# kluonj/HelFEM

Measured on AMD Instinct MI355X. Metric: scf_iteration_wall_time_fock_plus_geneig_nbf4230, lower is better.
Workload: dtype f64; 1 GPU; diatomic Z1=7 Z2=7 R=2.068 PBE, nelem=5 nnodes=15 nquad=75 lmmax=[20,20] (Nbf=4230, Nang=61, Nrad=70), XC grid 92x13, symmetry blocks [1380, 1470, 1380]: J+XC Fock build + eig_gsym_sub + density per step; parallelism=shard1, density=occupied orbitals of the core Hamiltonian

## Files before the change

helfem_amd/__init__.py:

```python
import ctypes
import os

import numpy as np

_HERE = os.path.dirname(os.path.abspath(__file__))
_LIB_PATH = os.environ.get("HELFEM_AMD_LIB") or os.path.join(_HERE, "lib", "libhelfem_amd.so")
_lib = None

c_double_p = ctypes.POINTER(ctypes.c_double)
c_int_p = ctypes.POINTER(ctypes.c_int)
c_i64_p = ctypes.POINTER(ctypes.c_int64)


class hfg_diatomic_desc(ctypes.Structure):
    _fields_ = [("Z1", ctypes.c_int), ("Z2", ctypes.c_int), ("Rhalf", ctypes.c_double), ("primbas", ctypes.c_int),
                ("nnodes", ctypes.c_int), ("nquad", ctypes.c_int), ("bval", c_double_p), ("nbval", ctypes.c_int),
                ("lval", c_int_p), ("mval", c_int_p), ("nang", ctypes.c_int), ("lpad", ctypes.c_int)]


class hfg_model_pot(ctypes.Structure):
    _fields_ = [("kind", ctypes.c_int), ("Z", ctypes.c_int), ("d", ctypes.c_double), ("H", ctypes.c_double)]


class hfg_atomic_desc(ctypes.Structure):
# ... 870 lines not shown

def xc_rs_kind(x_func):
    f = lib().hfg_xc_rs_kind
    f.argtypes = [ctypes.c_int]
    f.restype = ctypes.c_int
    return int(f(int(x_func)))


def scf_set_iguess(iguess):
    _check(lib().hfg_scf_set_iguess(int(iguess)))


def scf_diatomic(Z1, Z2, Rbond, lmmax, nelem, nnodes, method, nquad=0, Rmax=40.0, igrid=4, zexp=1.0, lpad=10, ldft=0,
                 mdft=0, symmetry=1, maxit=50, convthr=1e-7, verbose=0, ctx=None, M=1, occs=None, readocc=-1):
    ctx = ctx or default_context()
    L = lib()
    L.hfg_scf_diatomic.argtypes = [ctypes.c_void_p, ctypes.c_int, ctypes.c_int, ctypes.c_double, c_int_p, ctypes.c_int,
                                   ctypes.c_int, ctypes.c_int, ctypes.c_int, ctypes.c_double, ctypes.c_int,
                                   ctypes.c_double, ctypes.c_int, ctypes.c_char_p, ctypes.c_int, ctypes.c_int,
                                   ctypes.c_int, ctypes.c_int, ctypes.c_int, ctypes.c_double, ctypes.c_int, c_double_p]
    out = np.zeros(12)
    lm = (ctypes.c_int * len(lmmax))(*lmmax)
    scf_set_occupations(occs, readocc)
    try:
        _check(L.hfg_scf_diatomic(ctx.h, Z1, Z2, Rbond, lm, len(lmmax), nelem, nnodes, nquad, Rmax, igrid, zexp, lpad,
                                  method.encode(), ldft, mdft, symmetry, M, maxit, convthr, verbose, _p(out)))
    finally:
        scf_set_occupations(None)
    keys = ["Etot", "Ekin", "Epot", "Ecoul", "Exx", "Exc", "Enucr"]
    r = dict(zip(keys, out[:7]))
    r["iterations"] = int(out[7])
    r["converged"] = (out[7] - int(out[7])) > 0.25
    r["tJ"], r["tK"], r["tXC"], r["tdiag"] = out[8:12]
    return r


def scf_run_atomic(Z, lmax, mmax, nelem, nnodes, method="HF", ctx=None, check_only=False, E=None, C=None, extras=None, **kw):
    o = hfg_scf_options()
    _check(lib().hfg_scf_options_default(ctypes.byref(o), 1))
    o.Z1, o.lmax, o.mmax, o.nelem, o.nnodes = int(Z), int(lmax), int(mmax), int(nelem), int(nnodes)
    o.method = method.encode()
    o.verbose = 0
    o.save = b""
    for k, v in kw.items():
        if not hasattr(o, k):
            raise TypeError("hfg_scf_options has no field %s" % k)
        setattr(o, k, v.encode() if isinstance(v, str) else v)
    x = None
    if extras is not None:
        x = hfg_scf_atomic_extras()
        _check(lib().hfg_scf_atomic_extras_default(ctypes.byref(x)))
        for k, v in extras.items():
            if not hasattr(x, k):
                raise TypeError("hfg_scf_atomic_extras has no field %s" % k)
            setattr(x, k, v)
    xp = ctypes.byref(x) if x is not None else None
    if check_only:
        _check(lib().hfg_scf_options_check_ex(ctypes.byref(o), xp))
        return None
    ctx = ctx or default_context()
    r = hfg_scf_result()
    _check(lib().hfg_scf_run_ex(ctx.h, ctypes.byref(o), xp, ctypes.byref(r), _p(E) if E is not None else None,
                                _p(C) if C is not None else None))
    out = dict((f[0], getattr(r, f[0])) for f in hfg_scf_result._fields_)
    out["Econf"] = x.Econf if x is not None else 0.0
    return out


def scf_set_occupations(occs=None, readocc=-1):
    L = lib()
    L.hfg_scf_set_occupations.argtypes = [ctypes.c_int, ctypes.c_int, ctypes.c_int, ctypes.POINTER(ctypes.c_int)]
    if occs is None:
        _check(L.hfg_scf_set_occupations(0, 0, 0, None))
        return
    a = np.ascontiguousarray(np.asarray(occs, dtype=np.int32))
    _check(L.hfg_scf_set_occupations(int(readocc), a.shape[0], a.shape[1], a.ctypes.data_as(ctypes.POINTER(ctypes.c_int))))


def scf_atomic(Z, lmax, mmax, nelem, nnodes, method, Q=0, nquad=0, Rmax=40.0, igrid=4, zexp=2.0, ldft=0, mdft=0,
               symmetry=1, maxit=50, convthr=1e-7, verbose=0, ctx=None, M=1, maverage=False, occs=None, readocc=-1):
    ctx = ctx or default_context()
    L = lib()
    L.hfg_scf_atomic.argtypes = [ctypes.c_void_p] + [ctypes.c_int] * 7 + [ctypes.c_double, ctypes.c_int,
                                ctypes.c_double, ctypes.c_char_p] + [ctypes.c_int] * 6 + [ctypes.c_double,
                                ctypes.c_int, c_double_p]
    out = np.zeros(12)
    scf_set_occupations(occs, readocc)
    try:
        _check(L.hfg_scf_atomic(ctx.h, Z, Q, lmax, mmax, nelem, nnodes, nquad, Rmax, igrid, zexp, method.encode(), ldft,
                                mdft, symmetry, M, 1 if maverage else 0, maxit, convthr, verbose, _p(out)))
    finally:
        scf_set_occupations(None)
    keys = ["Etot", "Ekin", "Epot", "Ecoul", "Exx", "Exc", "Enucr"]
    r = dict(zip(keys, out[:7]))
    r["iterations"] = int(out[7])
    r["converged"] = (out[7] - int(out[7])) > 0.25
    r["tJ"], r["tK"], r["tXC"], r["tdiag"] = out[8:12]
    return r


class DeviceDIIS(object):

    def __init__(self, ctx, N, nspin, order=5, diiseps=1e-2, diisthr=1e-3, mode=0):
        self.h = None
        self.ctx, self.N, self.nspin, self.order, self.n = ctx, int(N), int(nspin), int(order), int(N)
        h = ctypes.c_void_p()
        _check(lib().hfg_diis_create(ctx.h, self.N, self.nspin, self.order, float(diiseps), float(diisthr), int(mode), ctypes.byref(h)))
        self.h = h

    def close(self):
        if self.h:
            if self.ctx.h:
                lib().hfg_diis_destroy(self.h)
            self.h = None

    def __del__(self):
        try:
            self.close()
        except Exception:
            pass

    @staticmethod
    def _dp(t):
        return ctypes.c_void_p(t.data_ptr()) if t is not None else None

    def _mat(self, t, cols, what):
        if t is None:
            return None
        if not (t.is_cuda and t.is_contiguous() and str(t.dtype) == "torch.float64" and t.numel() >= self.N * cols):
            raise ValueError("DeviceDIIS: %s must be a contiguous float64 tensor on the device with at least %d x %d elements"
                             % (what, self.N, cols))
        return t

    def set_metric(self, S, Sinvh):
        n = Sinvh.numel() // self.N
        if n * self.N != Sinvh.numel():
            raise ValueError("DeviceDIIS.set_metric: Sinvh is N x n")
        _check(lib().hfg_diis_set_metric_devptr(self.h, self._dp(self._mat(S, self.N, "S")), self._dp(self._mat(Sinvh, n, "Sinvh")), n))
        self.n = n

    def set_blocks(self, m_idx):
        ptr, idx = scf._blocks(m_idx or [])
        _check(lib().hfg_diis_set_blocks(self.h, len(m_idx or []), ptr.ctypes.data_as(c_i64_p), idx.ctypes.data_as(c_i64_p)))

    def update(self, E, Fa, Pa, Ca=None, nocca=0, Fb=None, Pb=None, Cb=None, noccb=0):
        if self.nspin == 2 and (Fb is None or Pb is None):
            raise ValueError("DeviceDIIS.update: nspin = 2 needs Fb and Pb")
        if self.nspin == 1 and (Fb is not None or Pb is not None):
            raise ValueError("DeviceDIIS.update: nspin = 1 takes one spin")
        err = ctypes.c_double()
        _check(lib().hfg_diis_update_devptr(self.h, float(E), self._dp(self._mat(Fa, self.N, "Fa")), self._dp(self._mat(Pa, self.N, "Pa")),
                                            self._dp(self._mat(Ca, int(nocca), "Ca")), int(nocca) if Ca is not None else 0,
                                            self._dp(self._mat(Fb, self.N, "Fb")), self._dp(self._mat(Pb, self.N, "Pb")),
                                            self._dp(self._mat(Cb, int(noccb), "Cb")), int(noccb) if Cb is not None else 0,
                                            ctypes.byref(err)))
        return err.value

    def solve(self, Fa, Fb=None):
        if self.nspin == 2 and Fb is None:
            raise ValueError("DeviceDIIS.solve: nspin = 2 needs Fb")
        dropped = ctypes.c_int()
        _check(lib().hfg_diis_solve_devptr(self.h, self._dp(self._mat(Fa, self.N, "Fa")), self._dp(self._mat(Fb, self.N, "Fb")),
                                           ctypes.byref(dropped)))
        return dropped.value

    @property
    def size(self):
        return int(lib().hfg_diis_size(self.h))

    def _get(self, which, count):
        out = np.zeros(max(count, 1))
        _check(lib().hfg_diis_get(self.h, which, _p(out), count))
        return out[:count]

    @property
    def B(self):
        k = self.size
        return self._get(0, k * k).reshape(k, k)

    @property
    def T(self):
        k = self.size
        return self._get(1, k * k).reshape(k, k)

    @property
    def weights(self):
        return self._get(2, self.size)

    @property
    def error(self):
        n = self.n
        return self._get(3, self.nspin * n * n).reshape(self.nspin, n, n).transpose(0, 2, 1)


def _refuse_out_of_scope(who, rohf, cuhf, readocc, maverage, dampfock):
    bad = [name for name, on in (("ROHF", rohf), ("CUHF", cuhf), ("readocc", readocc is not None and int(readocc) >= 0),
                                 ("maverage", maverage), ("dampfock", float(dampfock) != 1.0)) if on]
    if bad:
        raise NotImplementedError("%s.run: %s not supported by the step objects; use the SCF drivers (scf_diatomic, scf_atomic, "
                                  "scf_run_atomic)" % (who, ", ".join(bad)))


class DeviceSCFStep(object):

    def __init__(self, basis, x_func, c_func, ldft, mdft, nocc, symmetry=1, device=0, rank=0, nranks=1,
                 dens_thr=1e-12, kfrac=0.0, device_tei=False, fock_shard="auto"):
        self.nocc = int(nocc)
        self._setup(basis, x_func, c_func, ldft, mdft, symmetry, device, rank, nranks, dens_thr, kfrac, device_tei, fock_shard)
        f64 = dict(dtype=self.torch.float64, device=self.dev)
        L, N = lib(), self.N
        self.Fc = self.torch.zeros(int(L.hfg_fock_compact_size(basis.h)), **f64)
        self.scal = self.torch.zeros(3, **f64)
        self.F = self.torch.zeros(N * N, **f64)
        self.E = self.torch.zeros(N, **f64)
        self.C = self.torch.zeros(N * N, **f64)
        self.P = self.torch.zeros(N * N, **f64)
        nb = int(L.hfg_eig_block_buf_size(len(self.blocks), self.blk_ptr.ctypes.data_as(c_i64_p)))
        self.blockbuf = self.torch.zeros(nb, **f64)
        if self.kfrac != 0.0:
            self.K = self.torch.zeros(N * N, **f64)
            self.Pa = self.torch.zeros(N * N, **f64)

    def _setup(self, basis, x_func, c_func, ldft, mdft, symmetry, device, rank, nranks, dens_thr, kfrac, device_tei, fock_shard):
        import torch
        self.torch = torch
        self.basis = basis
        self.x_func, self.c_func, self.thr = int(x_func), int(c_func), float(dens_thr)
        self.dev = torch.device("cuda", device)
        torch.cuda.set_device(self.dev)
        self.ctx = Context(device, stream=torch.cuda.current_stream(self.dev).cuda_stream)
        self.ctx.set_shard(rank, nranks)
        self.rank, self.nranks = int(rank), int(nranks)
        self.fock_shard = os.environ.get("HELFEM_FOCK_SHARD", fock_shard)
        if device_tei:
            basis.compute_tei(float(kfrac) != 0.0, device=True, ctx=self.ctx)
        basis.upload(ldft, mdft, ctx=self.ctx)
        L = lib()
        L.hfg_fock_compact_size.restype = ctypes.c_int64
        L.hfg_eig_block_buf_size.restype = ctypes.c_int64
        L.hfg_fock_compact_dev.argtypes = [ctypes.c_void_p, ctypes.c_void_p, ctypes.c_int, ctypes.c_int, ctypes.c_void_p,
                                           ctypes.c_void_p, ctypes.c_void_p, ctypes.c_double]
        N = basis.Nbf()
        self.N = N
        self.blocks = basis.get_sym_idx(symmetry)
        self.blk_ptr, self.blk_idx = scf._blocks(self.blocks)
        blockid = np.zeros(N, dtype=np.int32)
        for ib, b in enumerate(self.blocks):
            blockid[b] = ib
        self.blockid = torch.from_numpy(blockid).to(self.dev)
        self.ctx.set_fock_blocks(basis, self.blockid.data_ptr())
        self.H0 = None
        self.Sinvh = None
        self.kfrac = float(kfrac)
        self.have_C = False
        self.have_density = False
        if self.kfrac != 0.0:
            L.hfg_exchange_occ_dev.argtypes = [ctypes.c_void_p, ctypes.c_void_p, ctypes.c_void_p, ctypes.c_void_p, ctypes.c_int64,
                                               ctypes.c_void_p]
            L.hfg_exchange_dev.argtypes = [ctypes.c_void_p, ctypes.c_void_p, ctypes.c_void_p, ctypes.c_void_p]

    def _ptr(self, t):
        return ctypes.c_void_p(t.data_ptr())

    def set_matrices(self, H0, Sinvh):
        t = self.torch
        self.H0 = t.from_numpy(np.asfortranarray(H0).ravel(order="F").copy()).to(self.dev)
        self.ctx.fix_sinvh(None)
        self.Sinvh = t.from_numpy(np.asfortranarray(Sinvh).ravel(order="F").copy()).to(self.dev)
        self.ctx.fix_sinvh(self.Sinvh.data_ptr())

    def set_density(self, P, C=None):
        self.P.copy_(self.torch.from_numpy(np.asfortranarray(P).ravel(order="F").copy()))
        self.have_density = True
        self.have_C = C is not None
        if C is not None:
            self.C[:self.N * self.nocc].copy_(self.torch.from_numpy(np.asfortranarray(C[:, :self.nocc]).ravel(order="F").copy()))

    def exchange(self):
        self.torch.mul(self.P, 0.5, out=self.Pa)
        if self.have_C:
            _check(lib().hfg_exchange_occ_dev(self.ctx.h, self.basis.h, self._ptr(self.Pa), self._ptr(self.C),
                                              ctypes.c_int64(self.nocc), self._ptr(self.K)))
        else:
            _check(lib().hfg_exchange_dev(self.ctx.h, self.basis.h, self._ptr(self.Pa), self._ptr(self.K)))

    def fock_partial(self):
        _check(lib().hfg_fock_compact_dev(self.ctx.h, self.basis.h, self.x_func, self.c_func, self._ptr(self.P),
                                          self._ptr(self.Fc), self._ptr(self.scal), self.thr))

    def fock_finish(self):
        _check(lib().hfg_fock_finish_dev(self.ctx.h, self.basis.h, self._ptr(self.Fc), self._ptr(self.H0),
                                         self._ptr(self.blockid), self._ptr(self.F)))

    def eig_partial(self):
        _check(lib().hfg_eig_blocks_dev(self.ctx.h, ctypes.c_int64(self.N), self._ptr(self.F), self._ptr(self.Sinvh),
                                        len(self.blocks), self.blk_ptr.ctypes.data_as(c_i64_p),
                                        self.blk_idx.ctypes.data_as(c_i64_p), self._ptr(self.blockbuf)))

    def eig_finish(self):
        _check(lib().hfg_eig_assemble_dev(self.ctx.h, ctypes.c_int64(self.N), len(self.blocks),
                                          self.blk_ptr.ctypes.data_as(c_i64_p), self.blk_idx.ctypes.data_as(c_i64_p),
                                          self._ptr(self.blockbuf), self._ptr(self.E), self._ptr(self.C)))

    def density(self):
        _check(lib().hfg_form_density_dev(self.ctx.h, ctypes.c_int64(self.N), ctypes.c_int64(self.N), self._ptr(self.C),
                                          ctypes.c_int64(self.nocc), self._ptr(self.P)))
        self.have_density = True

    def step(self, allreduce=None, exchange_blocks=None):
        shard_fock = self.nranks > 1 and self.fock_shard == "always"
        if self.nranks > 1 and not shard_fock:
            self.ctx.set_shard(0, 1)
        self.fock_partial()
        if self.nranks > 1 and not shard_fock:
            self.ctx.set_shard(self.rank, self.nranks)
        if allreduce is not None and (shard_fock or self.nranks == 1):
            allreduce(self.Fc)
            allreduce(self.scal)
        self.fock_finish()
        if self.kfrac != 0.0:
            self.exchange()
            if allreduce is not None:
                allreduce(self.K)
            self.F.add_(self.K, alpha=self.kfrac)
        self.eig_partial()
        if exchange_blocks is not None:
            exchange_blocks(self.blockbuf, len(self.blocks))
        elif allreduce is not None:
            allreduce(self.blockbuf)
        self.eig_finish()
        self.density()
        self.have_C = True

    def _whole_shard(self, fn):
        if self.nranks > 1:
            self.ctx.set_shard(0, 1)
        try:
            fn()
        finally:
            if self.nranks > 1:
                self.ctx.set_shard(self.rank, self.nranks)

    def _fock_stage(self, allreduce):
        shard_fock = self.nranks > 1 and self.fock_shard == "always"
        if shard_fock or self.nranks == 1:
            self.fock_partial()
            if allreduce is not None:
                allreduce(self.Fc)
                allreduce(self.scal)
        else:
            self._whole_shard(self.fock_partial)
        self.fock_finish()
        if self.kfrac != 0.0:
            self.exchange()
            if allreduce is not None:
                allreduce(self.K)
            self._add_exchange()

    def _add_exchange(self):
        self.F.add_(self.K, alpha=self.kfrac)

    def _eig_stage(self, allreduce, exchange_blocks):
        self.eig_partial()
        if exchange_blocks is not None:
            exchange_blocks(self.blockbuf, len(self.blocks))
        elif allreduce is not None:
            allreduce(self.blockbuf)
        self.eig_finish()

    def _coulomb_energy_matrix(self, P):
        if getattr(self, "J", None) is None:
            self.J = self.torch.zeros(self.N * self.N, dtype=self.torch.float64, device=self.dev)
        self._whole_shard(lambda: _check(lib().hfg_coulomb_dev(self.ctx.h, self.basis.h, self._ptr(P), self._ptr(self.J))))
        return self.J

    def _energy_terms(self):
        t = self.torch
        J = self._coulomb_energy_matrix(self.P)
        terms = [t.dot(self.P, self.H0), t.dot(self.P, J)]
        terms.append(t.dot(self.Pa, self.K) if self.kfrac != 0.0 else t.zeros((), dtype=t.float64, device=self.dev))
        return terms

    def energy(self, Enucr=0.0):
        t = self.torch
        v = t.stack(self._energy_terms() + [self.scal[0]]).cpu().numpy()
        r = dict(E1=float(v[0]), Ecoul=0.5 * float(v[1]), Exx=self._exx_factor() * float(v[2]), Exc=float(v[3]), Enucr=float(Enucr))
        r["Etot"] = r["E1"] + r["Ecoul"] + r["Exx"] + r["Exc"] + r["Enucr"]
        return r

    def _exx_factor(self):
        return self.kfrac

    def _nspin(self):
        return 1

    def _density_stage(self):
        self.density()
        self.P.mul_(2.0)
        self.have_C = True

    def _core_guess(self, allreduce, exchange_blocks):
        self.F.copy_(self.H0)
        self._eig_stage(allreduce, exchange_blocks)
        self._density_stage()

    def _diis_update(self, diis, E):
        if getattr(self, "Pa", None) is None:
            self.Pa = self.torch.zeros(self.N * self.N, dtype=self.torch.float64, device=self.dev)
        self.torch.mul(self.P, 0.5, out=self.Pa)
        if self.have_C:
            return diis.update(E, self.F, self.Pa, self.C, self.nocc)
        return diis.update(E, self.F, self.Pa)

    def _diis_solve(self, diis):
        diis.solve(self.F)

    def run(self, S, maxit=50, convthr=1e-7, Enucr=0.0, allreduce=None, exchange_blocks=None, diis=None, callback=None,
            rohf=False, cuhf=False, readocc=None, maverage=False, dampfock=1.0):
        _refuse_out_of_scope(type(self).__name__, rohf, cuhf, readocc, maverage, dampfock)
        if self.H0 is None:
            raise RuntimeError("run: set_matrices first")
        t = self.torch
        if diis is None:
            diis = DeviceDIIS(self.ctx, self.N, self._nspin())
            dS = t.from_numpy(np.asfortranarray(S, dtype=np.float64).ravel(order="F").copy()).to(self.dev)
            diis.set_metric(dS, self.Sinvh)
            if len(self.blocks) > 1:
                diis.set_blocks(self.blocks)
        if not self.have_density:
            self._core_guess(allreduce, exchange_blocks)
        trace, Eold, res, converged, it = [], 0.0, None, False, 0
        for it in range(1, int(maxit) + 1):
            self._fock_stage(allreduce)
            res = self.energy(Enucr)
            maxerr = self._diis_update(diis, res["Etot"])
            dE = res["Etot"] - Eold
            Eold = res["Etot"]
            trace.append((res["Etot"], maxerr))
            if callback is not None:
                callback(it, res["Etot"], maxerr)
            if maxerr < convthr and abs(dE) < convthr:
                converged = True
                break
            self._diis_solve(diis)
            self._eig_stage(allreduce, exchange_blocks)
            self._density_stage()
        res = dict(res or {})
        res.update(iterations=it, converged=converged, trace=trace)
        return res

    def numpy(self, t, shape):
        return t.cpu().numpy().reshape(shape, order="F")


class DeviceUSCFStep(DeviceSCFStep):

    def __init__(self, basis, x_func, c_func, ldft, mdft, nocc, symmetry=1, device=0, rank=0, nranks=1,
                 dens_thr=1e-12, kfrac=0.0, device_tei=False, fock_shard="auto"):
        self.nela, self.nelb = int(nocc[0]), int(nocc[1])
        if self.nela < 1 or self.nelb < 0:
            raise ValueError("DeviceUSCFStep: nocc = (nela >= 1, nelb >= 0)")
        self._setup(basis, x_func, c_func, ldft, mdft, symmetry, device, rank, nranks, dens_thr, kfrac, device_tei, fock_shard)
        t, N, L = self.torch, self.N, lib()
        f64 = dict(dtype=t.float64, device=self.dev)
        self.nc = int(L.hfg_fock_compact_size(basis.h))
        self.Fc = t.zeros(int(L.hfg_fock_compact_pol_size(basis.h)), **f64)
        self.scal = t.zeros(3, **f64)
        for name in ("Pa", "Pb", "Fa", "Fb", "Ca", "Cb"):
            setattr(self, name, t.zeros(N * N, **f64))
        self.Ea, self.Eb = t.zeros(N, **f64), t.zeros(N, **f64)
        if self.nranks > 1:
            nb = int(L.hfg_eig_block_buf_size(len(self.blocks), self.blk_ptr.ctypes.data_as(c_i64_p)))
            self.blockbuf_a, self.blockbuf_b = t.zeros(nb, **f64), t.zeros(nb, **f64)
        self.kbatch = False
        if self.kfrac != 0.0:
            self.K = t.zeros(2 * N * N, **f64)
            self.Ka, self.Kb = self.K[:N * N], self.K[N * N:]
            self.kbatch = {r["name"]: r["value"] for r in tuning_table()}["HELFEM_USCF_KBATCH"] == "on"
            if self.kbatch:
                self.Pab, self.Cab = t.zeros(2 * N * N, **f64), t.zeros(2 * N * N, **f64)
                self._nocc = np.array([self.nela, self.nelb], dtype=np.int64)

    def _spins(self):
        return ((self.Pa, self.Fa, self.Ea, self.Ca, self.nela), (self.Pb, self.Fb, self.Eb, self.Cb, self.nelb))

    def set_density(self, Pa, Pb, Ca=None, Cb=None):
        as_dev = lambda M: self.torch.from_numpy(np.asfortranarray(M).ravel(order="F").copy())
        self.Pa.copy_(as_dev(Pa))
        self.Pb.copy_(as_dev(Pb))
        self.have_density = True
        self.have_C = Ca is not None and (Cb is not None or self.nelb == 0)
        if self.have_C:
            self.Ca[:self.N * self.nela].copy_(as_dev(Ca[:, :self.nela]))
            if self.nelb:
                self.Cb[:self.N * self.nelb].copy_(as_dev(Cb[:, :self.nelb]))

    def exchange(self):
        if self.kbatch:
            N2 = self.N * self.N
            self.Pab[:N2].copy_(self.Pa)
            self.Pab[N2:].copy_(self.Pb)
            if self.have_C:
                self.Cab[:N2].copy_(self.Ca)
                self.Cab[N2:].copy_(self.Cb)
                _check(lib().hfg_exchange_occ_batch_devptr(self.ctx.h, self.basis.h, 2, self._ptr(self.Pab), self._ptr(self.Cab),
                                                           self._nocc.ctypes.data_as(c_i64_p), self.N, self._ptr(self.K)))
            else:
                _check(lib().hfg_exchange_batch_devptr(self.ctx.h, self.basis.h, 2, self._ptr(self.Pab), self._ptr(self.K)))
            return
        for (P, _, _, C, nocc), K in zip(self._spins(), (self.Ka, self.Kb)):
            if nocc == 0:
                K.zero_()
            elif self.have_C:
                _check(lib().hfg_exchange_occ_dev(self.ctx.h, self.basis.h, self._ptr(P), self._ptr(C), ctypes.c_int64(nocc),
                                                  self._ptr(K)))
            else:
                _check(lib().hfg_exchange_dev(self.ctx.h, self.basis.h, self._ptr(P), self._ptr(K)))

    def fock_partial(self):
        _check(lib().hfg_fock_compact_pol_devptr(self.ctx.h, self.basis.h, self.x_func, self.c_func, self._ptr(self.Pa),
                                                 self._ptr(self.Pb), self._ptr(self.Fc), self._ptr(self.scal), self.thr))

    def fock_finish(self):
        _check(lib().hfg_fock_finish_pol_devptr(self.ctx.h, self.basis.h, self._ptr(self.Fc), self._ptr(self.H0),
                                                self._ptr(self.blockid), self._ptr(self.Fa), self._ptr(self.Fb)))

    def eig_pair(self):
        _check(lib().hfg_eig_gsym_sub_pair_devptr(self.ctx.h, ctypes.c_int64(self.N), self._ptr(self.Fa), self._ptr(self.Fb),
                                                  self._ptr(self.Sinvh), len(self.blocks), self.blk_ptr.ctypes.data_as(c_i64_p),
                                                  self.blk_idx.ctypes.data_as(c_i64_p), self._ptr(self.Ea), self._ptr(self.Ca),
                                                  self._ptr(self.Eb), self._ptr(self.Cb)))

    def eig_partial(self):
        for (_, F, _, _, _), buf in zip(self._spins(), (self.blockbuf_a, self.blockbuf_b)):
            _check(lib().hfg_eig_blocks_dev(self.ctx.h, ctypes.c_int64(self.N), self._ptr(F), self._ptr(self.Sinvh),
                                            len(self.blocks), self.blk_ptr.ctypes.data_as(c_i64_p),
                                            self.blk_idx.ctypes.data_as(c_i64_p), self._ptr(buf)))

    def eig_finish(self):
        for (_, _, E, C, _), buf in zip(self._spins(), (self.blockbuf_a, self.blockbuf_b)):
            _check(lib().hfg_eig_assemble_dev(self.ctx.h, ctypes.c_int64(self.N), len(self.blocks),
                                              self.blk_ptr.ctypes.data_as(c_i64_p), self.blk_idx.ctypes.data_as(c_i64_p),
                                              self._ptr(buf), self._ptr(E), self._ptr(C)))

    def density(self):
        for P, _, _, C, nocc in self._spins():
            if nocc == 0:
                P.zero_()
                continue
            _check(lib().hfg_form_density_dev(self.ctx.h, ctypes.c_int64(self.N), ctypes.c_int64(self.N), self._ptr(C),
                                              ctypes.c_int64(nocc), self._ptr(P)))
        self.have_density = True

    def step(self, allreduce=None, exchange_blocks=None):
        shard_fock = self.nranks > 1 and self.fock_shard == "always"
        if self.nranks > 1 and not shard_fock:
            self.ctx.set_shard(0, 1)
        self.fock_partial()
        if self.nranks > 1 and not shard_fock:
            self.ctx.set_shard(self.rank, self.nranks)
        if allreduce is not None and (shard_fock or self.nranks == 1):
            allreduce(self.Fc)
            allreduce(self.scal)
        self.fock_finish()
        if self.kfrac != 0.0:
            self.exchange()
            if allreduce is not None:
                allreduce(self.K)
            self.Fa.add_(self.Ka, alpha=self.kfrac)
            self.Fb.add_(self.Kb, alpha=self.kfrac)
        if self.nranks == 1:
            self.eig_pair()
        else:
            self.eig_partial()
            for buf in (self.blockbuf_a, self.blockbuf_b):
                if exchange_blocks is not None:
                    exchange_blocks(buf, len(self.blocks))
                elif allreduce is not None:
                    allreduce(buf)
            self.eig_finish()
        self.density()
        self.have_C = True

    def _add_exchange(self):
        self.Fa.add_(self.Ka, alpha=self.kfrac)
        self.Fb.add_(self.Kb, alpha=self.kfrac)

    def _eig_stage(self, allreduce, exchange_blocks):
        if self.nranks == 1:
            self.eig_pair()
            return
        self.eig_partial()
        for buf in (self.blockbuf_a, self.blockbuf_b):
            if exchange_blocks is not None:
                exchange_blocks(buf, len(self.blocks))
            elif allreduce is not None:
                allreduce(buf)
        self.eig_finish()

    def _energy_terms(self):
        t = self.torch
        if getattr(self, "Pt", None) is None:
            self.Pt = t.zeros(self.N * self.N, dtype=t.float64, device=self.dev)
        t.add(self.Pa, self.Pb, out=self.Pt)
        J = self._coulomb_energy_matrix(self.Pt)
        terms = [t.dot(self.Pt, self.H0), t.dot(self.Pt, J)]
        terms.append(t.dot(self.Pa, self.Ka) + t.dot(self.Pb, self.Kb) if self.kfrac != 0.0
                     else t.zeros((), dtype=t.float64, device=self.dev))
        return terms

    def _exx_factor(self):
        return 0.5 * self.kfrac

    def _nspin(self):
        return 2

    def _density_stage(self):
        self.density()
        self.have_C = True

    def _core_guess(self, allreduce, exchange_blocks):
        self.Fa.copy_(self.H0)
        self.Fb.copy_(self.H0)
        self._eig_stage(allreduce, exchange_blocks)
        self._density_stage()

    def _diis_update(self, diis, E):
        if self.have_C:
            return diis.update(E, self.Fa, self.Pa, self.Ca, self.nela, self.Fb, self.Pb, self.Cb if self.nelb else None, self.nelb)
        return diis.update(E, self.Fa, self.Pa, Fb=self.Fb, Pb=self.Pb)

    def _diis_solve(self, diis):
        diis.solve(self.Fa, self.Fb)
```

helfem_amd/csrc/hip/common.h:

```cpp
#pragma once
#include <hip/hip_runtime.h>
#include <cstdint>
#include <cstring>
#include <map>
#include <stdexcept>
#include <string>
#include <vector>

#include "../../../include/helfem_gpu.h"
#include "../host/atomic_basis.h"
#include "../host/diatomic_basis.h"
#include "../host/tuning.h"
#include "workspace_owner.h"

namespace hfg {
using helfem::TrdMode, helfem::tuning;

void set_error(const std::string &msg);

#define HFG_HIP_CHECK(expr)                                                                          \
  do {                                                                                               \
    hipError_t _e = (expr);                                                                          \
    if (_e != hipSuccess)                                                                            \
      throw std::runtime_error(std::string("HIP error: ") + hipGetErrorString(_e) + " in " + #expr + \
                               " (" + __FILE__ + ":" + std::to_string(__LINE__) + ")");              \
  } while (0)

template <typename T>
struct DevBuf {
  T *p = nullptr;
  size_t n = 0;
  DevBuf() {}
  DevBuf(const DevBuf &) = delete;
  DevBuf &operator=(const DevBuf &) = delete;
  ~DevBuf() { release(); }
  void release() {
    if (p) (void)hipFree(p);
    p = nullptr;
    n = 0;
  }
  void resize(size_t count) {
    if (count <= n) return;
    release();
    HFG_HIP_CHECK(hipMalloc((void **)&p, count * sizeof(T)));
    n = count;
  }
  void upload(const std::vector<T> &h, hipStream_t s) {
    resize(h.size() ? h.size() : 1);
    if (h.size()) HFG_HIP_CHECK(hipMemcpyAsync(p, h.data(), h.size() * sizeof(T), hipMemcpyHostToDevice, s));
  }
};

template <typename T>
bool upload_cached(DevBuf<T> &buf, std::vector<T> &cache, const std::vector<T> &h, hipStream_t s) {
  if (buf.p && cache.size() == h.size() && buf.n >= h.size() &&
      (h.empty() || memcmp((const void *)cache.data(), (const void *)h.data(), h.size() * sizeof(T)) == 0))
    return false;
  HFG_HIP_CHECK(hipStreamSynchronize(s));
  cache = h;
  buf.upload(cache, s);
  return true;
}

struct ProfEntry {
  double ms = 0.0;
  int64_t launches = 0;
  std::vector<std::pair<hipEvent_t, hipEvent_t> > pending;
};

}

struct hfg_dev_tables;

struct hfg_ctx {
  int device = 0;
  hipStream_t stream = nullptr;
  bool own_stream = false;
  hipStream_t side_stream = nullptr;
  hipEvent_t side_ev[2] = {nullptr, nullptr};
  hipStream_t side();
  bool avoid_side = false;
  void drop_side();
  int shard_rank = 0, shard_n = 1;
  const double *fixed_sinvh = nullptr;
  unsigned long fixed_gen = 0;
  void fix_sinvh(const double *p) {
    fixed_sinvh = p;
    fixed_gen++;
  }
  hfg::DevBuf<int> fock_need, fock_gneed;
  const hfg_dev_tables *fock_need_tables = nullptr;
  int fock_need_A = 0, fock_need_G = 0;
  bool profiling = false;
  std::map<std::string, hfg::ProfEntry> prof;
  std::vector<hipEvent_t> event_pool;
  hfg::DevBuf<double> ws[8];
  double *pinned = nullptr;
  size_t pinned_bytes = 0;
  hfg::WorkspaceOwner<hfg::WS_CTX_SLOTS> work;

  void *pinned_buf(size_t bytes);
  hipEvent_t get_event();
  void prof_begin(const char *name);
  void prof_end(const char *name);
  void prof_collect();
};

struct hfg_basis {
  int kind = 0;
  helfem::diatomic::TwoDBasis b;
  helfem::atomic::TwoDBasis ab;
  hfg_dev_tables *dev = nullptr;
  hfg_dev_tables *dev_rs = nullptr;
  int dev_device = -1;
  hfg::DevBuf<double> dev_tei;
  bool tei_on_device = false;
  hfg::DevBuf<double> dev_rs_tei, dev_rs_disj;
  bool rs_on_device = false;

  size_t Nbf() const { return kind ? ab.Nbf() : b.Nbf(); }
  size_t Ndummy() const { return kind ? ab.Nbf() : b.Ndummy(); }
  size_t Nrad() const { return kind ? ab.Nrad() : b.Nrad(); }
  size_t Nang() const { return kind ? ab.Nang() : b.Nang(); }
  size_t Nel() const { return kind ? ab.Nel() : b.Nel(); }
  size_t max_Nprim() const { return kind ? ab.max_Nprim() : b.max_Nprim(); }
  bool have_tei() const { return tei_on_device || (kind ? ab.have_tei : b.have_tei); }
};

namespace hfg {
struct GemmTask {
  const double *A;
  const double *B;
  double *C;
  int M, N, K, lda, ldb, ldc;
  int tA = 0, tB = 0;
  double alpha = 1.0, beta = 0.0;
  int sym = 0;
  int over = 0;
  const int *amap = nullptr, *cmap = nullptr;
};
static_assert(sizeof(GemmTask) == 96, "GemmTask is compared bytewise: keep it free of padding");

struct ProfScope {
  hfg_ctx *c;
  const char *n;
  ProfScope(hfg_ctx *ctx, const char *name) : c(ctx), n(name) {
    if (c->profiling) c->prof_begin(n);
  }
  ~ProfScope() {
    if (c->profiling) c->prof_end(n);
  }
};
}
```

helfem_amd/csrc/hip/eig.hip:

```cpp
#include "internal.h"
#include "wave.h"
#include "../host/eigsel_count.h"
#include <cstdlib>
#include <cstring>

namespace hfg {

constexpr int MAXB = 8;
struct EigBatch {
  int nblk;
  int n[MAXB];
  double *A[MAXB];
  double *d[MAXB];
  double *e[MAXB];
  double *tau[MAXB];
  double *v[MAXB];
  double *pp[MAXB];
  double *dots[MAXB];
  double *Z[MAXB];
  int nz[MAXB];
  double *rot[MAXB];
  int *sweeps[MAXB];
  long rotcap[MAXB];
};

constexpr int TRD_NCS = 8;

__global__ void k_gather_block(const double *__restrict__ F, const double *__restrict__ S, int N,
                               const int64_t *__restrict__ rows, const int64_t *__restrict__ cols, int n,
                               double *__restrict__ Fb, double *__restrict__ Xb) {
  int i = blockIdx.x * blockDim.x + threadIdx.x;
  int j = blockIdx.y;
  if (i >= n) return;
  Fb[(size_t)j * n + i] = F[(size_t)rows[j] * N + rows[i]];
  Xb[(size_t)j * n + i] = S[(size_t)cols[j] * N + rows[i]];
}

__global__ void k_col_support(const double *__restrict__ S, int N, const int64_t *__restrict__ rows, int n,
                              int *__restrict__ flag) {
  int c = blockIdx.x;
  int any = 0;
  for (int i = threadIdx.x; i < n; i += blockDim.x)
    if (S[(size_t)c * N + rows[i]] != 0.0) any = 1;
  any = __syncthreads_or(any);
  if (threadIdx.x == 0) flag[c] = any;
}

__device__ inline void householder_of_column(const double *__restrict__ A, int n, int k, double *vsh, double *red,
                                             double &tau, double &beta) {
  const int m = n - k - 1;
  const double *x = A + (size_t)k * n + k + 1;
  double s = 0.0;
  for (int i = 1 + threadIdx.x; i < m; i += blockDim.x) s += x[i] * x[i];
  s = wave_sum(s);
  int nwave = blockDim.x / 64;
  if ((threadIdx.x & 63) == 0) red[threadIdx.x >> 6] = s;
  __syncthreads();
  double xn2 = 0.0;
  for (int w = 0; w < nwave; w++) xn2 += red[w];
  double alpha = x[0];
  double scale;
  if (xn2 == 0.0) {
    tau = 0.0;
    beta = alpha;
    scale = 0.0;
  } else {
    double nrm = sqrt(alpha * alpha + xn2);
    beta = (alpha >= 0.0) ? -nrm : nrm;
    tau = (beta - alpha) / beta;
    scale = 1.0 / (alpha - beta);
  }
  for (int i = threadIdx.x; i < m; i += blockDim.x) vsh[i] = (i == 0) ? 1.0 : x[i] * scale;
  __syncthreads();
}

__global__ __launch_bounds__(256) void k_trd_gemv(EigBatch b, int k) {
  extern __shared__ double sh[];
  const int blk = blockIdx.y;
  const int n = b.n[blk];
  if (k > n - 3) return;
  const int m = n - k - 1;
  const int nrs = (m + 63) / 64;
  const int rs = blockIdx.x / TRD_NCS, cs = blockIdx.x % TRD_NCS;
  if (rs >= nrs) return;
  double *A = b.A[blk];
  double *vsh = sh;
  double *red = sh + n;
  double tau, beta;
  householder_of_column(A, n, k, vsh, red, tau, beta);
  if (blockIdx.x == 0) {
    for (int i = threadIdx.x; i < m; i += blockDim.x) b.v[blk][i] = vsh[i];
    if (threadIdx.x == 0) {
      b.tau[blk][k] = tau;
      b.e[blk][k] = beta;
      b.d[blk][k] = A[(size_t)k * n + k];
    }
  }
  const int cchunk = (m + TRD_NCS - 1) / TRD_NCS;
  const int c0 = cs * cchunk, c1 = min(m, c0 + cchunk);
  const int wave = threadIdx.x >> 6, lane = threadIdx.x & 63;
  const int row = rs * 64 + lane;
  double acc = 0.0;
  if (row < m) {
    const double *a = A + (size_t)(k + 1) * n + (k + 1) + row;
    for (int c = c0 + wave; c < c1; c += 4) acc += a[(size_t)c * n] * vsh[c];
  }
  __syncthreads();
  red[wave * 64 + lane] = acc;
  __syncthreads();
  if (wave == 0) {
    double p = red[lane] + red[64 + lane] + red[128 + lane] + red[192 + lane];
    if (row < m) b.pp[blk][(size_t)cs * n + row] = p;
    double dv = (row < m) ? p * vsh[row] : 0.0;
    dv = wave_sum(dv);
    if (lane == 0) b.dots[blk][blockIdx.x] = dv;
  }
}

__global__ __launch_bounds__(256) void k_trd_update(EigBatch b, int k) {
  __shared__ double vr[64], vc[64], wr[64], wc[64];
  __shared__ double Ksh;
  const int blk = blockIdx.y;
  const int n = b.n[blk];
  if (k > n - 3) return;
  const int m = n - k - 1;
  const int nt = (m + 63) / 64;
  if ((int)blockIdx.x >= nt * nt) return;
  const int tr = blockIdx.x % nt, tc = blockIdx.x / nt;
  double *A = b.A[blk];
  const double tau = b.tau[blk][k];
  if (threadIdx.x == 0) {
    const int nrs = (m + 63) / 64;
    double s = 0.0;
    for (int i = 0; i < nrs * TRD_NCS; i++) s += b.dots[blk][i];
    Ksh = 0.5 * tau * tau * s;
  }
  __syncthreads();
  if (threadIdx.x < 128) {
    int which = threadIdx.x >> 6, l = threadIdx.x & 63;
    int idx = (which ? tc : tr) * 64 + l;
    double v = 0.0, w = 0.0;
    if (idx < m) {
      v = b.v[blk][idx];
      double p = 0.0;
      for (int cs = 0; cs < TRD_NCS; cs++) p += b.pp[blk][(size_t)cs * n + idx];
      w = tau * p - Ksh * v;
    }
    if (which) {
      vc[l] = v;
      wc[l] = w;
    } else {
      vr[l] = v;
      wr[l] = w;
    }
  }
  __syncthreads();
  const int lane = threadIdx.x & 63, wave = threadIdx.x >> 6;
  const int row = tr * 64 + lane;
  if (row < m) {
    double *a = A + (size_t)(k + 1) * n + (k + 1) + row;
    for (int c = wave; c < 64; c += 4) {
      int col = tc * 64 + c;
      if (col < m) a[(size_t)col * n] -= vr[lane] * wc[c] + wr[lane] * vc[c];
    }
  }
  if (blockIdx.x == 0) {
    for (int i = 1 + threadIdx.x; i < m; i += blockDim.x) A[(size_t)k * n + k + 1 + i] = b.v[blk][i];
  }
}

__global__ void k_trd_finish(EigBatch b) {
  int blk = blockIdx.x;
  if (threadIdx.x != 0) return;
  int n = b.n[blk];
  double *A = b.A[blk];
  if (n >= 2) {
    b.d[blk][n - 2] = A[(size_t)(n - 2) * n + (n - 2)];
    b.e[blk][n - 2] = A[(size_t)(n - 2) * n + (n - 1)];
    b.tau[blk][n - 2] = 0.0;
  }
  b.d[blk][n - 1] = A[(size_t)(n - 1) * n + (n - 1)];
  b.e[blk][n - 1] = 0.0;
}

__global__ void k_tql_values(EigBatch b) {
  int blk = blockIdx.x;
  if (threadIdx.x != 0) return;
  const int n = b.n[blk];
  double *d = b.d[blk], *e = b.e[blk];
  double *rot = b.rot[blk];
  int *sw = b.sweeps[blk];
  long nrot = 0;
  int nsw = 0;
  int status = 0;
  const long cap = b.rotcap[blk];
  for (int l = 0; l < n && !status; l++) {
    int iter = 0;
    int m;
    do {
      for (m = l; m + 1 < n; m++) {
        double dd = fabs(d[m]) + fabs(d[m + 1]);
        if (fabs(e[m]) <= 2.220446049250313e-16 * dd) break;
      }
      if (m != l) {
        if (iter++ == 300) {
          status = 1;
          break;
        }
        if (nrot + (m - l) > cap || 4 * (nsw + 1) + 2 >= 4 * 64 * n) {
          status = 2;
          break;
        }
        double g = (d[l + 1] - d[l]) / (2.0 * e[l]);
        double r = hypot(g, 1.0);
        g = d[m] - d[l] + e[l] / (g + (g >= 0.0 ? fabs(r) : -fabs(r)));
        double s = 1.0, c = 1.0, p = 0.0;
        int cnt = 0;
        bool under = false;
        int i;
        for (i = m - 1; i >= l; i--) {
          double f = s * e[i], bb = c * e[i];
          r = hypot(f, g);
          e[i + 1] = r;
          if (r == 0.0) {
            d[i + 1] -= p;
            e[m] = 0.0;
            under = true;
            break;
          }
          s = f / r;
          c = g / r;
          g = d[i + 1] - p;
          r = (d[i] - g) * s + 2.0 * c * bb;
          p = s * r;
          d[i + 1] = g + p;
          g = c * r - bb;
          rot[2 * (nrot + cnt)] = c;
          rot[2 * (nrot + cnt) + 1] = s;
          cnt++;
        }
        sw[2 + 4 * nsw + 0] = l;
        sw[2 + 4 * nsw + 1] = m;
        sw[2 + 4 * nsw + 2] = (int)(nrot & 0x7fffffff);
        sw[2 + 4 * nsw + 3] = cnt;
        nsw++;
        nrot += cnt;
        if (under) continue;
        d[l] -= p;
        e[l] = g;
        e[m] = 0.0;
      }
    } while (m != l);
  }
  sw[0] = nsw;
  sw[1] = status;
}

__global__ void k_set_identity(EigBatch b) {
  int blk = blockIdx.z;
  int n = b.n[blk];
  int i = blockIdx.x * blockDim.x + threadIdx.x, j = blockIdx.y;
  if (i < n && j < n) b.Z[blk][(size_t)j * n + i] = (i == j) ? 1.0 : 0.0;
}

__global__ void k_tql_apply(EigBatch b) {
  int blk = blockIdx.y;
  int n = b.n[blk];
  int k = blockIdx.x * blockDim.x + threadIdx.x;
  if (k >= n) return;
  double *Z = b.Z[blk] + k;
  const double *rot = b.rot[blk];
  const int *sw = b.sweeps[blk];
  int nsw = sw[0];
  long off = 0;
  for (int q = 0; q < nsw; q++) {
    int m = sw[2 + 4 * q + 1], cnt = sw[2 + 4 * q + 3];
    double hi = Z[(size_t)m * n];
    int i = m - 1;
    for (int t = 0; t < cnt; t++, i--) {
      double c = rot[2 * (off + t)], s = rot[2 * (off + t) + 1];
      double lo = Z[(size_t)i * n];
      Z[(size_t)(i + 1) * n] = s * lo + c * hi;
      hi = c * lo - s * hi;
    }
    Z[(size_t)(i + 1) * n] = hi;
    off += cnt;
  }
}

template <int NR>
__global__ __launch_bounds__(256) void k_backtransform(EigBatch b) {
  int blk = blockIdx.y;
  int n = b.n[blk];
  int col = blockIdx.x * 4 + (threadIdx.x >> 6);
  int lane = threadIdx.x & 63;
  if (col >= b.nz[blk]) return;
  const double *A = b.A[blk];
  const double *tau = b.tau[blk];
  double *z = b.Z[blk] + (size_t)col * n;
  double zr[NR];
#pragma unroll
  for (int r = 0; r < NR; r++) {
    int i = lane + 64 * r;
    zr[r] = (i < n) ? z[i] : 0.0;
  }
  for (int k = n - 3; k >= 0; k--) {
    double t = tau[k];
    if (t == 0.0) continue;
    const double *v = A + (size_t)k * n;
    double s = 0.0;
    double vr[NR];
#pragma unroll
    for (int r = 0; r < NR; r++) {
      int i = lane + 64 * r;
      double vi = 0.0;
      if (i == k + 1) vi = 1.0;
      else if (i > k + 1 && i < n) vi = v[i];
      vr[r] = vi;
      s += vi * zr[r];
    }
    s = wave_sum(s);
    s *= t;
#pragma unroll
    for (int r = 0; r < NR; r++) zr[r] -= s * vr[r];
  }
#pragma unroll
  for (int r = 0; r < NR; r++) {
    int i = lane + 64 * r;
    if (i < n) z[i] = zr[r];
  }
}

__global__ __launch_bounds__(256) void k_backtransform_lds(EigBatch b) {
  extern __shared__ double sh[];
  int blk = blockIdx.y;
  int n = b.n[blk];
  int wave = threadIdx.x >> 6, lane = threadIdx.x & 63;
  int col = blockIdx.x * 4 + wave;
  if (col >= b.nz[blk]) return;
  const double *A = b.A[blk];
  const double *tau = b.tau[blk];
  double *z = b.Z[blk] + (size_t)col * n;
  double *zs = sh + (size_t)wave * n;
  for (int i = lane; i < n; i += 64) zs[i] = z[i];
  for (int k = n - 3; k >= 0; k--) {
    double t = tau[k];
    if (t == 0.0) continue;
    const double *v = A + (size_t)k * n;
    double s = 0.0;
    for (int i = k + 1 + lane; i < n; i += 64) s += ((i == k + 1) ? 1.0 : v[i]) * zs[i];
    s = wave_sum(s);
    s *= t;
    for (int i = k + 1 + lane; i < n; i += 64) zs[i] -= s * ((i == k + 1) ? 1.0 : v[i]);
  }
  for (int i = lane; i < n; i += 64) z[i] = zs[i];
}

constexpr int RANK_SEG = 8;
__global__ __launch_bounds__(256) void k_rank(const double *__restrict__ E, int n, int *__restrict__ rank) {
  __shared__ double sE[256];
  const int i = blockIdx.x * 256 + threadIdx.x;
  const double ei = (i < n) ? E[i] : 0.0;
  const int seg = (n + RANK_SEG - 1) / RANK_SEG;
  const int j0 = blockIdx.y * seg, j1 = min(n, j0 + seg);
  int r = 0;
  for (int c = j0; c < j1; c += 256) {
    __syncthreads();
    sE[threadIdx.x] = (c + (int)threadIdx.x < j1) ? E[c + threadIdx.x] : 0.0;
    __syncthreads();
    const int m = min(256, j1 - c);
    if (m == 256) {
#pragma unroll 16
      for (int jj = 0; jj < 256; jj++) {
        const double ej = sE[jj];
        r += (ej < ei) || (ej == ei && c + jj < i);
      }
    } else {
      for (int jj = 0; jj < m; jj++) {
        const double ej = sE[jj];
        r += (ej < ei) || (ej == ei && c + jj < i);
      }
    }
  }
  if (i < n && r) atomicAdd(&rank[i], r);
}
static void launch_rank(hfg_ctx *ctx, const double *E, int n, int *rank) {
  HFG_HIP_CHECK(hipMemsetAsync(rank, 0, sizeof(int) * n, ctx->stream));
  hipLaunchKernelGGL(k_rank, dim3((n + 255) / 256, RANK_SEG), dim3(256), 0, ctx->stream, E, n, rank);
}

__global__ void k_scatter_cols(const double *__restrict__ Cb, int nrow, int ncol, const int64_t *__restrict__ rows,
                               const int *__restrict__ rank, int coff, const double *__restrict__ Eb, int ldc,
                               double *__restrict__ Cout, double *__restrict__ Eout) {
  int i = blockIdx.x * blockDim.x + threadIdx.x;
  int j = blockIdx.y;
  if (i >= nrow) return;
  int c = rank[coff + j];
  size_t r = rows ? (size_t)rows[i] : (size_t)i;
  Cout[(size_t)c * ldc + r] = Cb[(size_t)j * nrow + i];
  if (i == 0) Eout[c] = Eb[j];
}

__global__ void k_take_lowest(const double *__restrict__ Z, const double *__restrict__ E, int n, int nev, const int *__restrict__ rank,
                              double *__restrict__ Zs, double *__restrict__ Ws) {
  int i = blockIdx.x * blockDim.x + threadIdx.x;
  int j = blockIdx.y;
  int c = rank[j];
  if (i >= n || c >= nev) return;
  Zs[(size_t)c * n + i] = Z[(size_t)j * n + i];
  if (i == 0) Ws[c] = E[j];
}

constexpr int BT_KB = 64;

__global__ void k_bt_extract(EigBatch b, double *const *__restrict__ Vx) {
  const int blk = blockIdx.z;
  const int n = b.n[blk];
  const int j = blockIdx.y;
  const int g = blockIdx.x * blockDim.x + threadIdx.x;
  if (j >= n || g >= n) return;
  double v = 0.0;
  if (j <= n - 3) {
    if (g == j + 1) v = 1.0;
    else if (g > j + 1) v = b.A[blk][(size_t)j * n + g];
  }
  Vx[blk][(size_t)j * n + g] = v;
}

constexpr int BT_PW = 2 * BT_KB;
constexpr int BT_WREP = 4;
__global__ __launch_bounds__(256) void k_bt_wpair(EigBatch b, double *const *__restrict__ Wpart, double *const *__restrict__ W,
                                                  double *const *__restrict__ Cc, int S, int GS, int npair, int pair,
                                                  int mirror) {
  __shared__ double sC[BT_KB][BT_KB + 1];
  __shared__ double s1[4][BT_KB];
  const int blk = blockIdx.y;
  const int n = b.n[blk];
  const int j0 = pair * BT_PW;
  if (j0 > n - 3) return;
  const int kb1 = min(BT_KB, n - 2 - (j0 + BT_KB));
  const int tid = threadIdx.x, cl = tid >> 6, i = tid & 63;
  if (kb1 > 0) {
    constexpr int NE = BT_KB * BT_KB / 256;
    double c[NE];
#pragma unroll
    for (int u = 0; u < NE; u++) c[u] = 0.0;
    for (int sl = 0; sl < GS; sl++) {
      const double *src = Cc[blk] + ((size_t)sl * npair + pair) * BT_KB * BT_KB + tid;
#pragma unroll
      for (int u = 0; u < NE; u++) c[u] += src[256 * u];
    }
#pragma unroll
    for (int u = 0; u < NE; u++) {
      const int t = tid + 256 * u;
      sC[t % BT_KB][t / BT_KB] = c[u];
    }
  }
  const size_t tot = (size_t)BT_PW * n;
  double a0[BT_WREP], a1[BT_WREP];
#pragma unroll
  for (int rep = 0; rep < BT_WREP; rep++) {
    const int col = (blockIdx.x * BT_WREP + rep) * 4 + cl;
    a0[rep] = 0.0;
    a1[rep] = 0.0;
    if (col < n) {
      for (int sl = 0; sl < S; sl++) {
        a0[rep] += Wpart[blk][(size_t)sl * tot + (size_t)col * BT_PW + i];
        a1[rep] += Wpart[blk][(size_t)sl * tot + (size_t)col * BT_PW + BT_KB + i];
      }
    }
  }
  if (mirror) {
    const int kb0 = min(BT_KB, n - 2 - j0);
#pragma unroll
    for (int rep = 0; rep < BT_WREP; rep++) {
      const int col = (blockIdx.x * BT_WREP + rep) * 4 + cl;
      __syncthreads();
      s1[cl][i] = (i < kb0) ? a0[rep] : 0.0;
      __syncthreads();
      if (col < n) {
        double r1 = 0.0;
        if (kb1 > 0 && i < kb1) {
          double corr = 0.0;
          for (int j = 0; j < kb0; j++) corr += sC[j][i] * s1[cl][j];
          r1 = a1[rep] - corr;
        }
        W[blk][(size_t)col * BT_PW + i] = a0[rep];
        W[blk][(size_t)col * BT_PW + BT_KB + i] = r1;
      }
    }
    return;
  }
#pragma unroll
  for (int rep = 0; rep < BT_WREP; rep++) {
    const int col = (blockIdx.x * BT_WREP + rep) * 4 + cl;
    __syncthreads();
    s1[cl][i] = (kb1 > 0 && i < kb1) ? a1[rep] : 0.0;
    __syncthreads();
    if (col < n) {
      double r0 = a0[rep];
      if (kb1 > 0) {
        double corr = 0.0;
        for (int j = 0; j < kb1; j++) corr += sC[i][j] * s1[cl][j];
        r0 -= corr;
      }
      W[blk][(size_t)col * BT_PW + i] = r0;
      W[blk][(size_t)col * BT_PW + BT_KB + i] = (kb1 > 0 && i < kb1) ? a1[rep] : 0.0;
    }
  }
}

constexpr int BT_GS = 4;
__global__ __launch_bounds__(64) void k_bt_T(EigBatch b, double *const *__restrict__ G, double *const *__restrict__ T,
                                             int P) {
  __shared__ double sT[BT_KB][BT_KB + 1];
  __shared__ double sG[BT_KB][BT_KB + 1];
  __shared__ double sg[BT_KB];
  const int blk = blockIdx.y, p = blockIdx.x;
  const int n = b.n[blk];
  const int j0 = p * BT_KB;
  if (j0 > n - 3) return;
  const int kb = min(BT_KB, n - 2 - j0);
  double *Tp = T[blk] + (size_t)p * BT_KB * BT_KB;
  const int t = threadIdx.x;
  for (int c0 = 0; c0 < BT_KB; c0 += 16) {
    double g[16];
#pragma unroll
    for (int u = 0; u < 16; u++) g[u] = 0.0;
#pragma unroll
    for (int sl = 0; sl < BT_GS; sl++) {
      const double *src = G[blk] + ((size_t)sl * P + p) * BT_KB * BT_KB + (size_t)c0 * BT_KB + t;
#pragma unroll
      for (int u = 0; u < 16; u++) g[u] += src[(size_t)u * BT_KB];
    }
#pragma unroll
    for (int u = 0; u < 16; u++) {
      sG[c0 + u][t] = g[u];
      sT[t][c0 + u] = 0.0;
    }
  }
  __shared__ double stau[BT_KB];
  stau[t] = (t < kb) ? b.tau[blk][j0 + t] : 0.0;
  __syncthreads();
  for (int i = 0; i < kb; i++) {
    const double ti = stau[i];
    sg[t] = (t < i) ? sG[i][t] : 0.0;
    __syncthreads();
    if (t < i) {
      double acc0 = 0.0, acc1 = 0.0, acc2 = 0.0, acc3 = 0.0;
#pragma unroll
      for (int k = 0; k < BT_KB; k += 4) {
        acc0 += sT[t][k] * sg[k];
        acc1 += sT[t][k + 1] * sg[k + 1];
        acc2 += sT[t][k + 2] * sg[k + 2];
        acc3 += sT[t][k + 3] * sg[k + 3];
      }
      sT[t][i] = -ti * ((acc0 + acc1) + (acc2 + acc3));
    }
    if (t == i) sT[i][i] = ti;
    __syncthreads();
  }
  for (int c = 0; c < BT_KB; c++) Tp[(size_t)c * BT_KB + t] = sT[t][c];
}

struct EigWork : Workspace {
  GemmHow full_how;
  std::vector<int64_t> asm_rows;
  DevBuf<long long> asm_rows_dev;
  bool folded = false;
  DevBuf<double> Y[MAXB];
  DevBuf<GemmTask> btslabR, btupdR;
  std::vector<GemmTask> h_btslabR, h_btupdR;
  DevBuf<double> A[MAXB], d[MAXB], e[MAXB], tau[MAXB], v[MAXB], pp[MAXB], dots[MAXB], Z[MAXB], rot[MAXB];
  DevBuf<double> Zs[MAXB], Ws[MAXB];
  DevBuf<int> selrank;
  DevBuf<int> sweeps[MAXB];
  DevBuf<int> ibuf1, ibuf2;
  DevBuf<GemmTask> gtasks, bttasks, btslab, btgram, btcpl, btupd;
  std::vector<GemmTask> h_gtasks, h_bttasks, h_btslab, h_btgram, h_btcpl, h_btupd;
  std::vector<double *> h_btptr;
  DevBuf<double> Vx[MAXB], G[MAXB], T[MAXB], VT[MAXB], Wb[MAXB], Wp[MAXB], Cc[MAXB];
  DevBuf<double *> btptr;
  bool used_dc = true;
  DevBuf<double> idx;
  const double *sup_S = nullptr;
  unsigned long sup_gen = 0;
  int sup_N = 0;
  std::vector<int64_t> sup_ptr, sup_idx;
};
static EigWork &work_for(hfg_ctx *ctx) { return ctx->work.get<EigWork>(WS_EIG); }

struct CopySlices {
  const double *src[16];
  double *dst[16];
  int n[16];
};
__global__ void k_copy_slices(CopySlices c) {
  const int q = blockIdx.y;
  for (int i = blockIdx.x * blockDim.x + threadIdx.x; i < c.n[q]; i += gridDim.x * blockDim.x) c.dst[q][i] = c.src[q][i];
}
static void copy_slices(hipStream_t s, const std::vector<const double *> &src, const std::vector<double *> &dst, const std::vector<int> &n) {
  for (size_t q0 = 0; q0 < src.size(); q0 += 16) {
    CopySlices c{};
    const int m = (int)std::min<size_t>(16, src.size() - q0);
    int nmax = 0;
    for (int q = 0; q < m; q++) {
      c.src[q] = src[q0 + q];
      c.dst[q] = dst[q0 + q];
      c.n[q] = n[q0 + q];
      nmax = std::max(nmax, n[q0 + q]);
    }
    if (nmax > 0) hipLaunchKernelGGL(k_copy_slices, dim3((nmax + 255) / 256, m), dim3(256), 0, s, c);
  }
}

struct TrPtrs {
  const double *src[MAXB];
  double *dst[MAXB];
  int n[MAXB];
};
__global__ __launch_bounds__(256) void k_transpose_batch(TrPtrs t) {
  __shared__ double tile[64][65];
  const int blk = blockIdx.z, n = t.n[blk];
  const int bi = blockIdx.x * 64, bj = blockIdx.y * 64;
  if (bi >= n || bj >= n) return;
  const int tx = threadIdx.x & 63, ty = threadIdx.x >> 6;
  for (int c = ty; c < 64; c += 4) {
    const int gm = bi + tx, gn = bj + c;
    tile[c][tx] = (gm < n && gn < n) ? t.src[blk][(size_t)gn * n + gm] : 0.0;
  }
  __syncthreads();
  for (int c = ty; c < 64; c += 4) {
    const int gm = bj + tx, gn = bi + c;
    if (gm < n && gn < n) t.dst[blk][(size_t)gn * n + gm] = tile[tx][c];
  }
}

static void bt_wy_setup(hfg_ctx *ctx, EigWork &w, const EigBatch &b, int nblk, const int *ns, int nmax, bool fold = false) {
  hipStream_t s = ctx->stream;
  const int P = (nmax - 3) / BT_KB + 1;
  const int NP = (P + 1) / 2;
  constexpr int BT_S = 6;
  std::vector<double *> ptrs(6 * (size_t)nblk);
  for (int k = 0; k < nblk; k++) {
    const int n = ns[k];
    w.Vx[k].resize((size_t)n * n);
    w.G[k].resize((size_t)BT_GS * P * BT_KB * BT_KB);
    w.T[k].resize((size_t)P * BT_KB * BT_KB);
    w.VT[k].resize((size_t)n * P * BT_KB);
    w.Wb[k].resize((size_t)BT_PW * n);
    w.Wp[k].resize((size_t)BT_S * BT_PW * n);
    w.Cc[k].resize((size_t)BT_GS * NP * BT_KB * BT_KB);
    ptrs[k] = w.Vx[k].p;
    ptrs[nblk + k] = w.G[k].p;
    ptrs[2 * nblk + k] = w.T[k].p;
    ptrs[3 * nblk + k] = w.Wp[k].p;
    ptrs[4 * nblk + k] = w.Wb[k].p;
    ptrs[5 * nblk + k] = w.Cc[k].p;
  }
  upload_cached(w.btptr, w.h_btptr, ptrs, s);
  GemmTask none;
  none.A = none.B = nullptr;
  none.C = nullptr;
  none.M = none.N = none.K = 0;
  none.lda = none.ldb = none.ldc = 1;
  auto kb_of = [&](int k, int p) { return std::max(0, std::min(BT_KB, ns[k] - 2 - p * BT_KB)); };
  auto chunk_of = [](int len, int parts) { return ((len + parts - 1) / parts + 15) / 16 * 16; };

  std::vector<GemmTask> gram((size_t)BT_GS * P * nblk, none), vt((size_t)P * nblk, none);
  for (int p = 0; p < P; p++)
    for (int k = 0; k < nblk; k++) {
      const int n = ns[k], j0 = p * BT_KB, kb = kb_of(k, p);
      if (kb <= 0) continue;
      const int r0 = j0 + 1, mr = n - r0;
      const double *Vp = w.Vx[k].p + (size_t)j0 * n + r0;
      const int chunk = chunk_of(mr, BT_GS);
      for (int sl = 0; sl < BT_GS; sl++) {
        GemmTask g = none;
        const int k0 = sl * chunk, kk = std::max(0, std::min(chunk, mr - k0));
        g.A = g.B = Vp + (kk > 0 ? k0 : 0);
        g.C = w.G[k].p + ((size_t)sl * P + p) * BT_KB * BT_KB;
        g.tA = 1;
        g.M = g.N = kb;
        g.K = kk;
        g.lda = g.ldb = n;
        g.ldc = BT_KB;
        gram[((size_t)sl * P + p) * nblk + k] = g;
      }
      const int rp = (p & ~1) * BT_KB + 1;
      GemmTask g = none;
      g.A = w.Vx[k].p + (size_t)j0 * n + rp;
      g.B = w.T[k].p + (size_t)p * BT_KB * BT_KB;
      g.C = w.VT[k].p + (size_t)j0 * n + rp;
      g.M = n - rp;
      g.N = g.K = kb;
      g.lda = n;
      g.ldb = BT_KB;
      g.ldc = n;
      vt[(size_t)p * nblk + k] = g;
    }
  upload_cached(w.btgram, w.h_btgram, gram, s);
  upload_cached(w.bttasks, w.h_bttasks, vt, s);

  std::vector<GemmTask> cpl((size_t)BT_GS * NP * nblk, none), slab((size_t)NP * BT_S * nblk, none), upd((size_t)NP * nblk, none);
  for (int g2 = 0; g2 < NP; g2++)
    for (int k = 0; k < nblk; k++) {
      const int n = ns[k], p0 = 2 * g2, j0 = p0 * BT_KB;
      const int kb0 = kb_of(k, p0), kb1 = (p0 + 1 < P) ? kb_of(k, p0 + 1) : 0;
      if (kb0 <= 0) continue;
      const int r0 = j0 + 1, mr = n - r0, kbp = kb0 + kb1;
      if (kb1 > 0) {
        const int r1 = j0 + BT_KB + 1, m1 = n - r1;
        const int chunk = chunk_of(m1, BT_GS);
        for (int sl = 0; sl < BT_GS; sl++) {
          GemmTask c = none;
          const int k0 = sl * chunk, kk = std::max(0, std::min(chunk, m1 - k0));
          c.A = w.Vx[k].p + (size_t)j0 * n + r1 + (kk > 0 ? k0 : 0);
          c.B = w.VT[k].p + (size_t)(j0 + BT_KB) * n + r1 + (kk > 0 ? k0 : 0);
          c.C = w.Cc[k].p + ((size_t)sl * NP + g2) * BT_KB * BT_KB;
          c.tA = 1;
          c.M = kb0;
          c.N = kb1;
          c.K = kk;
          c.lda = c.ldb = n;
          c.ldc = BT_KB;
          cpl[((size_t)sl * NP + g2) * nblk + k] = c;
        }
      }
      const int chunk = chunk_of(mr, BT_S);
      for (int sl = 0; sl < BT_S; sl++) {
        GemmTask q = none;
        const int k0 = sl * chunk, kk = std::max(0, std::min(chunk, mr - k0));
        q.A = w.Vx[k].p + (size_t)j0 * n + r0 + (kk > 0 ? k0 : 0);
        q.B = b.Z[k] + r0 + (kk > 0 ? k0 : 0);
        q.C = w.Wp[k].p + (size_t)sl * BT_PW * n;
        q.tA = 1;
        q.M = kbp;
        q.N = b.nz[k];
        q.K = kk;
        q.lda = q.ldb = n;
        q.ldc = BT_PW;
        slab[((size_t)g2 * BT_S + sl) * nblk + k] = q;
      }
      GemmTask u = none;
      u.A = w.VT[k].p + (size_t)j0 * n + r0;
      u.B = w.Wb[k].p;
      u.C = b.Z[k] + r0;
      u.M = mr;
      u.N = b.nz[k];
      u.K = kbp;
      u.lda = n;
      u.ldb = BT_PW;
      u.ldc = n;
      u.alpha = -1.0;
      u.beta = 1.0;
      upd[(size_t)g2 * nblk + k] = u;
    }
  upload_cached(w.btcpl, w.h_btcpl, cpl, s);
  upload_cached(w.btslab, w.h_btslab, slab, s);
  upload_cached(w.btupd, w.h_btupd, upd, s);
  if (fold) {
    std::vector<GemmTask> slabR((size_t)NP * BT_S * nblk, none), updR((size_t)NP * nblk, none);
    for (int g2 = 0; g2 < NP; g2++)
      for (int k = 0; k < nblk; k++) {
        const int n = ns[k], p0 = 2 * g2, j0 = p0 * BT_KB;
        const int kb0 = kb_of(k, p0), kb1 = (p0 + 1 < P) ? kb_of(k, p0 + 1) : 0;
        if (kb0 <= 0) continue;
        const int r0 = j0 + 1, mr = n - r0, kbp = kb0 + kb1;
        const int chunk = chunk_of(mr, BT_S);
        for (int sl = 0; sl < BT_S; sl++) {
          GemmTask q = none;
          const int k0 = sl * chunk, kk = std::max(0, std::min(chunk, mr - k0));
          q.A = w.VT[k].p + (size_t)j0 * n + r0 + (kk > 0 ? k0 : 0);
          q.B = w.Y[k].p + r0 + (kk > 0 ? k0 : 0);
          q.C = w.Wp[k].p + (size_t)sl * BT_PW * n;
          q.tA = 1;
          q.M = kbp;
          q.N = n;
          q.K = kk;
          q.lda = q.ldb = n;
          q.ldc = BT_PW;
          slabR[((size_t)g2 * BT_S + sl) * nblk + k] = q;
        }
        GemmTask u = none;
        u.A = w.Vx[k].p + (size_t)j0 * n + r0;
        u.B = w.Wb[k].p;
        u.C = w.Y[k].p + r0;
        u.M = mr;
        u.N = n;
        u.K = kbp;
        u.lda = n;
        u.ldb = BT_PW;
        u.ldc = n;
        u.alpha = -1.0;
        u.beta = 1.0;
        updR[(size_t)g2 * nblk + k] = u;
      }
    upload_cached(w.btslabR, w.h_btslabR, slabR, s);
    upload_cached(w.btupdR, w.h_btupdR, updR, s);
  }
}

static void bt_wy_prepare(hfg_ctx *ctx, EigWork &w, const EigBatch &b, int nblk, int nmax, bool on_side = false) {
  const int P = (nmax - 3) / BT_KB + 1;
  const bool use_side = (tuning().bt_side && !ctx->avoid_side) || on_side;
  hipStream_t main = ctx->stream, q = main;
  const bool prof = ctx->profiling;
  if (use_side) {
    q = ctx->side();
    HFG_HIP_CHECK(hipEventRecord(ctx->side_ev[0], main));
    HFG_HIP_CHECK(hipStreamWaitEvent(q, ctx->side_ev[0], 0));
    ctx->profiling = false;
    ctx->stream = q;
  }
  try {
    double *const *dptr = w.btptr.p;
    hipLaunchKernelGGL(k_bt_extract, dim3((nmax + 255) / 256, nmax, nblk), dim3(256), 0, q, b, dptr);
    gemm_tasklist_dev(ctx, w.btgram.p, BT_GS * P * nblk, BT_KB, BT_KB, {GemmTile::T64});
    hipLaunchKernelGGL(k_bt_T, dim3(P, nblk), dim3(BT_KB), 0, q, b, dptr + nblk, dptr + 2 * nblk, P);
    gemm_tasklist_dev(ctx, w.bttasks.p, P * nblk, nmax, BT_KB, {GemmTile::T64});
    gemm_tasklist_dev(ctx, w.btcpl.p, BT_GS * ((P + 1) / 2) * nblk, BT_KB, BT_KB, {GemmTile::T64});
  } catch (...) {
    ctx->stream = main;
    ctx->profiling = prof;
    throw;
  }
  ctx->stream = main;
  ctx->profiling = prof;
  if (use_side) HFG_HIP_CHECK(hipEventRecord(ctx->side_ev[1], q));
}

static void bt_wy_apply(hfg_ctx *ctx, EigWork &w, const EigBatch &b, int nblk, int nmax) {
  hipStream_t s = ctx->stream;
  const int P = (nmax - 3) / BT_KB + 1, NP = (P + 1) / 2;
  constexpr int BT_S = 6;
  double *const *dptr = w.btptr.p;
  if (tuning().bt_side && !ctx->avoid_side) HFG_HIP_CHECK(hipStreamWaitEvent(s, ctx->side_ev[1], 0));
  for (int g = NP - 1; g >= 0; g--) {
    gemm_tasklist_dev(ctx, w.btslab.p + (size_t)g * BT_S * nblk, BT_S * nblk, BT_PW, nmax, {GemmTile::T64});
    hipLaunchKernelGGL(k_bt_wpair, dim3((nmax + 4 * BT_WREP - 1) / (4 * BT_WREP), nblk), dim3(256), 0, s, b, dptr + 3 * nblk, dptr + 4 * nblk,
                       dptr + 5 * nblk, BT_S, BT_GS, NP, g, 0);
    gemm_tasklist_dev(ctx, w.btupd.p + (size_t)g * nblk, nblk, nmax, nmax, {tuning().acc_tile != 128 ? GemmTile::T64 : GemmTile::T128,  true});
  }
  HFG_HIP_CHECK(hipGetLastError());
}

static void bt_wy_fold_x(hfg_ctx *ctx, EigWork &w, const EigBatch &b, int nblk, const int *ns, int nmax, const double *const *X) {
  const int P = (nmax - 3) / BT_KB + 1, NP = (P + 1) / 2;
  constexpr int BT_S = 6;
  hipStream_t main = ctx->stream, q = ctx->side();
  const bool prof = ctx->profiling;
  ctx->profiling = false;
  ctx->stream = q;
  try {
    TrPtrs t;
    for (int k = 0; k < MAXB; k++) {
      t.src[k] = k < nblk ? X[k] : nullptr;
      t.dst[k] = k < nblk ? w.Y[k].p : nullptr;
      t.n[k] = k < nblk ? ns[k] : 0;
    }
    hipLaunchKernelGGL(k_transpose_batch, dim3((nmax + 63) / 64, (nmax + 63) / 64, nblk), dim3(256), 0, q, t);
    double *const *dptr = w.btptr.p;
    for (int g = 0; g < NP; g++) {
      gemm_tasklist_dev(ctx, w.btslabR.p + (size_t)g * BT_S * nblk, BT_S * nblk, BT_PW, nmax, {GemmTile::T64});
      hipLaunchKernelGGL(k_bt_wpair, dim3((nmax + 4 * BT_WREP - 1) / (4 * BT_WREP), nblk), dim3(256), 0, q, b, dptr + 3 * nblk, dptr + 4 * nblk,
                         dptr + 5 * nblk, BT_S, BT_GS, NP, g, 1);
      gemm_tasklist_dev(ctx, w.btupdR.p + (size_t)g * nblk, nblk, nmax, nmax, {GemmTile::T64,  true});
    }
  } catch (...) {
    ctx->stream = main;
    ctx->profiling = prof;
    throw;
  }
  ctx->stream = main;
  ctx->profiling = prof;
  HFG_HIP_CHECK(hipGetLastError());
  HFG_HIP_CHECK(hipEventRecord(ctx->side_ev[1], q));
}

constexpr double EIGSEL_CROSS = 0.0;
static bool eigsel_takes_stein(int nblk, const int *ns, const int *nev) {
  const helfem::EigSel how = tuning().eigsel;
  if (how != helfem::EigSel::crossover) return how == helfem::EigSel::stein;
  long want = 0, all = 0;
  for (int i = 0; i < nblk; i++) {
    want += nev[i];
    all += ns[i];
  }
  return (double)want <= EIGSEL_CROSS * (double)all;
}
static void eig_sym_batch(hfg_ctx *ctx, EigWork &w, int nblk, const int *ns, const double *const *foldX = nullptr,
                          const int *nev = nullptr) {
  EigBatch b;
  b.nblk = nblk;
  int nmax = 0, nzmax = 0;
  const bool stein = nev && eigsel_takes_stein(nblk, ns, nev);
  for (int i = 0; i < nblk; i++) {
    int n = ns[i];
    nmax = std::max(nmax, n);
    b.n[i] = n;
    b.nz[i] = nev ? nev[i] : n;
    nzmax = std::max(nzmax, b.nz[i]);
    if (nev) {
      if (nev[i] < 1 || nev[i] > n) throw std::logic_error("eig_sym_batch: 1 <= nev <= n violated\n");
      w.Zs[i].resize((size_t)n * nev[i]);
      w.Ws[i].resize(nev[i]);
    }
    w.d[i].resize(n);
    w.e[i].resize(n);
    w.tau[i].resize(n);
    w.v[i].resize(n);
    w.pp[i].resize((size_t)TRD_NCS * n);
    w.dots[i].resize((size_t)TRD_NCS * ((n + 63) / 64) + 8);
    if (!stein) w.Z[i].resize((size_t)n * n);
    long cap = 3L * n * n + 1024;
    w.rot[i].resize(2 * (size_t)cap);
    w.sweeps[i].resize((size_t)4 * 64 * n + 8);
    b.rotcap[i] = cap;
    b.A[i] = w.A[i].p;
    b.d[i] = w.d[i].p;
    b.e[i] = w.e[i].p;
    b.tau[i] = w.tau[i].p;
    b.v[i] = w.v[i].p;
    b.pp[i] = w.pp[i].p;
    b.dots[i] = w.dots[i].p;
    b.Z[i] = stein ? nullptr : w.Z[i].p;
    b.rot[i] = w.rot[i].p;
    b.sweeps[i] = w.sweeps[i].p;
  }
  hipStream_t s = ctx->stream;
  const bool bt_wy = !tuning().bt_column && nmax >= 4 * BT_KB;
  if (tridiagonalize_takes_chain(nblk, ns)) {
    ctx->avoid_side = true;
    ctx->drop_side();
  }
  const bool fold = bt_wy && foldX != nullptr && tuning().bt_fold && !ctx->avoid_side;
  w.folded = fold;
  if (fold)
    for (int i = 0; i < nblk; i++) w.Y[i].resize((size_t)ns[i] * ns[i]);
  EigBatch bz = b;
  if (nev)
    for (int i = 0; i < nblk; i++) bz.Z[i] = w.Zs[i].p;
  if (bt_wy) bt_wy_setup(ctx, w, bz, nblk, ns, nmax, fold);
  {
    ProfScope ps(ctx, "eig_tridiag");
    if (tuning().trd_mode == TrdMode::unblocked) {
      size_t shb = (size_t)(nmax + 4 * 64 + 8) * sizeof(double);
      if (shb > 64 * 1024)
        HFG_HIP_CHECK(hipFuncSetAttribute((const void *)k_trd_gemv, hipFuncAttributeMaxDynamicSharedMemorySize, (int)shb));
      for (int k = 0; k <= nmax - 3; k++) {
        int m = nmax - k - 1;
        int nrs = (m + 63) / 64;
        hipLaunchKernelGGL(k_trd_gemv, dim3(nrs * TRD_NCS, nblk), dim3(256), shb, s, b, k);
        hipLaunchKernelGGL(k_trd_update, dim3(nrs * nrs, nblk), dim3(256), 0, s, b, k);
      }
      hipLaunchKernelGGL(k_trd_finish, dim3(nblk), dim3(64), 0, s, b);
    } else {
      double *Ap[MAXB], *dp[MAXB], *ep[MAXB], *tp[MAXB];
      for (int i = 0; i < nblk; i++) {
        Ap[i] = w.A[i].p;
        dp[i] = w.d[i].p;
        ep[i] = w.e[i].p;
        tp[i] = w.tau[i].p;
      }
      tridiagonalize_batch(ctx, nblk, ns, Ap, dp, ep, tp);
    }
  }
  if (bt_wy) bt_wy_prepare(ctx, w, b, nblk, nmax, fold);
  if (fold) bt_wy_fold_x(ctx, w, b, nblk, ns, nmax, foldX);
  if (stein) {
    ProfScope ps(ctx, "eig_tridiag_sel");
    w.used_dc = true;
    double *dp[MAXB], *ep[MAXB], *wp[MAXB], *zp[MAXB];
    for (int i = 0; i < nblk; i++) {
      dp[i] = w.d[i].p;
      ep[i] = w.e[i].p;
      wp[i] = w.Ws[i].p;
      zp[i] = w.Zs[i].p;
    }
    tridiag_sel_batch(ctx, nblk, ns, nev, dp, ep, wp, zp);
  } else {
    ProfScope ps(ctx, "eig_tridiag_solve");
    w.used_dc = !tuning().tridiag_ql;
    if (!w.used_dc) {
      hipLaunchKernelGGL(k_set_identity, dim3((nmax + 255) / 256, nmax, nblk), dim3(256), 0, s, b);
      hipLaunchKernelGGL(k_tql_values, dim3(nblk), dim3(64), 0, s, b);
      hipLaunchKernelGGL(k_tql_apply, dim3((nmax + 63) / 64, nblk), dim3(64), 0, s, b);
    } else {
      double *dp[MAXB], *ep[MAXB], *zp[MAXB];
      for (int i = 0; i < nblk; i++) {
        dp[i] = w.d[i].p;
        ep[i] = w.e[i].p;
        zp[i] = w.Z[i].p;
      }
      tridiag_dc_batch(ctx, nblk, ns, dp, ep, zp);
    }
    if (nev) {
      size_t off = 0;
      for (int i = 0; i < nblk; i++) off += ns[i] + 8;
      w.selrank.resize(off);
      off = 0;
      for (int i = 0; i < nblk; i++) {
        launch_rank(ctx, w.d[i].p, ns[i], w.selrank.p + off);
        hipLaunchKernelGGL(k_take_lowest, dim3((ns[i] + 255) / 256, ns[i]), dim3(256), 0, s, w.Z[i].p, w.d[i].p, ns[i], nev[i],
                           w.selrank.p + off, w.Zs[i].p, w.Ws[i].p);
        off += ns[i] + 8;
      }
    }
  }
  {
    ProfScope ps(ctx, "eig_backtransform");
    if (fold) {
      HFG_HIP_CHECK(hipStreamWaitEvent(s, ctx->side_ev[1], 0));
    } else if (bt_wy) {
      bt_wy_apply(ctx, w, bz, nblk, nmax);
    } else {
    dim3 grid((nzmax + 3) / 4, nblk);
    if (nmax <= 64 * 8)
      hipLaunchKernelGGL(k_backtransform<8>, grid, dim3(256), 0, s, bz);
    else if (nmax <= 64 * 24)
      hipLaunchKernelGGL(k_backtransform<24>, grid, dim3(256), 0, s, bz);
    else {
      size_t shb = (size_t)4 * nmax * sizeof(double);
      if (shb > 64 * 1024)
        HFG_HIP_CHECK(
            hipFuncSetAttribute((const void *)k_backtransform_lds, hipFuncAttributeMaxDynamicSharedMemorySize, (int)shb));
      hipLaunchKernelGGL(k_backtransform_lds, grid, dim3(256), shb, s, bz);
    }
    }
  }
  HFG_HIP_CHECK(hipGetLastError());
}

static void check_status(hfg_ctx *ctx, EigWork &w, int nblk) {
  if (w.used_dc) {
    if (dc_status(ctx) != 0) throw std::logic_error("Eigendecomposition failed!\n");
    trdp_check_status(ctx);
    return;
  }
  for (int i = 0; i < nblk; i++) {
    int st[2];
    HFG_HIP_CHECK(hipMemcpyAsync(st, w.sweeps[i].p, 2 * sizeof(int), hipMemcpyDeviceToHost, ctx->stream));
    HFG_HIP_CHECK(hipStreamSynchronize(ctx->stream));
    if (st[1] != 0) throw std::logic_error("Eigendecomposition failed!\n");
  }
}

void eig_sym_dev(hfg_ctx *ctx, int n, const double *dA, double *dE, double *dC) {
  EigWork &w = work_for(ctx);
  w.A[0].resize((size_t)n * n + 2);
  HFG_HIP_CHECK(hipMemcpyAsync(w.A[0].p, dA, sizeof(double) * n * n, hipMemcpyDeviceToDevice, ctx->stream));
  eig_sym_batch(ctx, w, 1, &n);
  DevBuf<int> &rank = w.ibuf1;
  rank.resize(n + 8);
  launch_rank(ctx, w.d[0].p, n, rank.p);
  hipLaunchKernelGGL(k_scatter_cols, dim3((n + 255) / 256, n), dim3(256), 0, ctx->stream, w.Z[0].p, n, n,
                     (const int64_t *)nullptr, rank.p, 0, w.d[0].p, n, dC, dE);
  check_status(ctx, w, 1);
}

void eig_sym_sel_dev(hfg_ctx *ctx, int n, const double *dA, int nev, double *dE, double *dC) {
  if (nev < 1) throw std::logic_error("eig_sym_sel: nev must be at least 1\n");
  if (n < 1) throw std::logic_error("eig_sym_sel: empty matrix\n");
  nev = std::min(nev, n);
  EigWork &w = work_for(ctx);
  w.A[0].resize((size_t)n * n + 2);
  HFG_HIP_CHECK(hipMemcpyAsync(w.A[0].p, dA, sizeof(double) * n * n, hipMemcpyDeviceToDevice, ctx->stream));
  eig_sym_batch(ctx, w, 1, &n, nullptr, &nev);
  HFG_HIP_CHECK(hipMemcpyAsync(dC, w.Zs[0].p, sizeof(double) * (size_t)n * nev, hipMemcpyDeviceToDevice, ctx->stream));
  HFG_HIP_CHECK(hipMemcpyAsync(dE, w.Ws[0].p, sizeof(double) * nev, hipMemcpyDeviceToDevice, ctx->stream));
  check_status(ctx, w, 1);
}

void eig_gsym_dev(hfg_ctx *ctx, int N, int n, const double *dF, const double *dS, double *dE, double *dC) {
  EigWork &w = work_for(ctx);
  w.A[0].resize((size_t)n * n + 2);
  DevBuf<double> &T1 = ctx->ws[0];
  DevBuf<double> &Ctmp = ctx->ws[1];
  T1.resize((size_t)N * n);
  Ctmp.resize((size_t)N * n);
  {
    ProfScope ps(ctx, "eig_reduce");
    gemm_dev(ctx, false, false, N, n, N, 1.0, dF, N, dS, N, 0.0, T1.p, N);
    gemm_dev(ctx, true, false, n, n, N, 1.0, dS, N, T1.p, N, 0.0, w.A[0].p, n);
  }
  eig_sym_batch(ctx, w, 1, &n);
  {
    ProfScope ps(ctx, "eig_backtransform");
    gemm_dev(ctx, false, false, N, n, n, 1.0, dS, N, w.Z[0].p, n, 0.0, Ctmp.p, N);
  }
  DevBuf<int> &rank = w.ibuf1;
  rank.resize(n + 8);
  launch_rank(ctx, w.d[0].p, n, rank.p);
  hipLaunchKernelGGL(k_scatter_cols, dim3((N + 255) / 256, n), dim3(256), 0, ctx->stream, Ctmp.p, N, n,
                     (const int64_t *)nullptr, rank.p, 0, w.d[0].p, N, dC, dE);
  check_status(ctx, w, 1);
}

size_t eig_block_buf_size(int nblk, const int64_t *blk_ptr) {
  size_t nmax = 0;
  for (int ib = 0; ib < nblk; ib++) nmax = std::max<size_t>(nmax, blk_ptr[ib + 1] - blk_ptr[ib]);
  return (size_t)nblk * (nmax * nmax + nmax);
}

static void eig_blocks_multi_dev(hfg_ctx *ctx, int N, int nF, const double *const *dFs, const double *dS, int nblk, const int64_t *blk_ptr,
                                 const int64_t *blk_idx, double *const *dBlockBufs, int nev = 0);
static int eig_num_cus(hfg_ctx *ctx) {
  static const int ncu = [&] {
    hipDeviceProp_t prop;
    return (hipGetDeviceProperties(&prop, ctx->device) == hipSuccess && prop.multiProcessorCount > 0) ? prop.multiProcessorCount : 256;
  }();
  return ncu;
}
void eig_blocks_dev(hfg_ctx *ctx, int N, const double *dF, const double *dS, int nblk, const int64_t *blk_ptr,
                    const int64_t *blk_idx, double *dBlockBuf) {
  eig_blocks_multi_dev(ctx, N, 1, &dF, dS, nblk, blk_ptr, blk_idx, &dBlockBuf);
}
static void eig_blocks_multi_dev(hfg_ctx *ctx, int N, int nF, const double *const *dFs, const double *dS, int nblk, const int64_t *blk_ptr,
                                 const int64_t *blk_idx, double *const *dBlockBufs, int nev) {
  EigWork &w = work_for(ctx);
  hipStream_t s = ctx->stream;
  if (blk_ptr[nblk] != N) throw std::logic_error("Symmetry mismatch in eig_gsym_sub\n");
  DevBuf<double> &idxbuf = w.idx;
  idxbuf.resize(2 * (size_t)N + 16);
  int64_t *drows = (int64_t *)idxbuf.p;
  int64_t *dcols = drows + N;
  for (int ib = 0; ib < nblk; ib++)
    if (blk_ptr[ib + 1] == blk_ptr[ib]) throw std::logic_error("eig_gsym_sub: empty symmetry block\n");
  const bool cached = ctx->fixed_sinvh && ctx->fixed_sinvh == dS && w.sup_S == dS && w.sup_gen == ctx->fixed_gen &&
                      w.sup_N == N &&
                      w.sup_ptr.size() == (size_t)nblk + 1 && std::equal(w.sup_ptr.begin(), w.sup_ptr.end(), blk_ptr) &&
                      w.sup_idx.size() == (size_t)N && std::equal(w.sup_idx.begin(), w.sup_idx.end(), blk_idx);
  if (!cached) {
    w.sup_S = nullptr;
    HFG_HIP_CHECK(hipMemcpyAsync(drows, blk_idx, sizeof(int64_t) * N, hipMemcpyHostToDevice, s));
    DevBuf<int> &flag = w.ibuf2;
    flag.resize((size_t)N * nblk + 8);
    for (int ib = 0; ib < nblk; ib++) {
      int n = (int)(blk_ptr[ib + 1] - blk_ptr[ib]);
      hipLaunchKernelGGL(k_col_support, dim3(N), dim3(256), 0, s, dS, N, drows + blk_ptr[ib], n, flag.p + (size_t)ib * N);
    }
    std::vector<int> hflag((size_t)N * nblk);
    HFG_HIP_CHECK(hipMemcpyAsync(hflag.data(), flag.p, sizeof(int) * hflag.size(), hipMemcpyDeviceToHost, s));
    HFG_HIP_CHECK(hipStreamSynchronize(s));
    std::vector<int64_t> allcols;
    for (int ib = 0; ib < nblk; ib++) {
      int cnt = 0;
      for (int c = 0; c < N; c++)
        if (hflag[(size_t)ib * N + c]) {
          allcols.push_back(c);
          cnt++;
        }
      if (cnt != (int)(blk_ptr[ib + 1] - blk_ptr[ib]))
        throw std::logic_error("eig_gsym_sub: Sinvh is not block structured (columns with support != block size)\n");
    }
    HFG_HIP_CHECK(hipMemcpyAsync(dcols, allcols.data(), sizeof(int64_t) * N, hipMemcpyHostToDevice, s));
    HFG_HIP_CHECK(hipStreamSynchronize(s));
    if (ctx->fixed_sinvh == dS) {
      w.sup_S = dS;
      w.sup_gen = ctx->fixed_gen;
      w.sup_N = N;
      w.sup_ptr.assign(blk_ptr, blk_ptr + nblk + 1);
      w.sup_idx.assign(blk_idx, blk_idx + N);
    }
  }

  size_t nmax = 0;
  for (int ib = 0; ib < nblk; ib++) nmax = std::max<size_t>(nmax, blk_ptr[ib + 1] - blk_ptr[ib]);
  const size_t slot = nmax * nmax + nmax;
  for (int f = 0; f < nF; f++) HFG_HIP_CHECK(hipMemsetAsync(dBlockBufs[f], 0, sizeof(double) * slot * nblk, s));

  std::vector<int> mine;
  for (int f = 0; f < nF; f++)
    for (int ib = 0; ib < nblk; ib++)
      if (ib % ctx->shard_n == ctx->shard_rank) mine.push_back(f * nblk + ib);
  DevBuf<double> &Fb = ctx->ws[5];
  DevBuf<double> &T1 = ctx->ws[0];
  DevBuf<double> &Xall = ctx->ws[4];
  Fb.resize(nmax * nmax * MAXB);
  T1.resize(nmax * nmax * MAXB);
  Xall.resize(nmax * nmax * MAXB);
  for (size_t c0 = 0; c0 < mine.size(); c0 += MAXB) {
    int nb = (int)std::min<size_t>(MAXB, mine.size() - c0);
    std::vector<int> ns(nb), nevs(nb);
    std::vector<GemmTask> gt(4 * (size_t)nb);
    const double *Xptr[MAXB];
    int nm = 0;
    for (int k = 0; k < nb; k++) {
      const int ib = mine[c0 + k] % nblk;
      double *dBlockBuf = dBlockBufs[mine[c0 + k] / nblk];
      int n = (int)(blk_ptr[ib + 1] - blk_ptr[ib]);
      ns[k] = n;
      nevs[k] = nev > 0 ? std::min(nev, n) : n;
      nm = std::max(nm, n);
      w.A[k].resize((size_t)n * n + 2);
      if (nev > 0) w.Zs[k].resize((size_t)n * nevs[k]);
      else w.Z[k].resize((size_t)n * n);
      w.Y[k].resize((size_t)n * n);
      double *Xb = Xall.p + (size_t)k * nmax * nmax, *Fk = Fb.p + (size_t)k * nmax * nmax, *Tk = T1.p + (size_t)k * nmax * nmax;
      Xptr[k] = Xb;
      GemmTask g;
      g.M = g.N = g.K = n;
      g.lda = g.ldb = g.ldc = n;
      g.A = Fk;
      g.B = Xb;
      g.C = Tk;
      gt[k] = g;
      g.A = Xb;
      g.tA = 1;
      g.B = Tk;
      g.C = w.A[k].p;
      g.sym = 1;
      gt[nb + k] = g;
      g.sym = 0;
      g.tA = 0;
      g.A = Xb;
      g.B = nev > 0 ? w.Zs[k].p : w.Z[k].p;
      g.N = nevs[k];
      g.C = dBlockBuf + (size_t)ib * slot;
      gt[2 * nb + k] = g;
      g.A = w.Y[k].p;
      g.tA = 1;
      gt[3 * nb + k] = g;
    }
    upload_cached(w.gtasks, w.h_gtasks, gt, s);
    {
      ProfScope ps(ctx, "eig_reduce");
      for (int k = 0; k < nb; k++) {
        const int ib = mine[c0 + k] % nblk;
        const double *dF = dFs[mine[c0 + k] / nblk];
        int n = ns[k];
        hipLaunchKernelGGL(k_gather_block, dim3((n + 255) / 256, n), dim3(256), 0, s, dF, dS, N, drows + blk_ptr[ib],
                           dcols + blk_ptr[ib], n, Fb.p + (size_t)k * nmax * nmax, Xall.p + (size_t)k * nmax * nmax);
      }
      const int force_split = tuning().gemm_splitk;
      long full_tiles = 0, low_tiles = 0;
      for (int k = 0; k < nb; k++) {
        const long t1 = (ns[k] + 127) / 128;
        full_tiles += t1 * t1;
        low_tiles += t1 * (t1 + 1) / 2;
      }
      const int slots = 2 * eig_num_cus(ctx);
      const bool split_full = force_split >= 0 ? force_split != 0 : (full_tiles < slots && nm >= 256);
      const bool split_low = force_split >= 0 ? force_split != 0 : (low_tiles < slots && nm >= 256);
      ProfScope pp3(ctx, "eig_products");
      const bool tile64 = force_split < 0 && !gemm_prefers_128(ctx, full_tiles);
      GemmHow full, low;
      if (tile64) full.tile = low.tile = GemmTile::T64;
      else {
        if (split_full) full.tile = GemmTile::T128, full.split2 = true;
        else if (tuning().gemm_rect) full.tile = GemmTile::T128x64;
        if (split_low) low.tile = GemmTile::T128, low.split2 = true;
      }
      w.full_how = full;
      if (full.split2)
        for (int k = 0; k < nb; k++) HFG_HIP_CHECK(hipMemsetAsync(T1.p + (size_t)k * nmax * nmax, 0, sizeof(double) * (size_t)ns[k] * ns[k], s));
      gemm_tasklist_dev(ctx, w.gtasks.p, nb, nm, nm, full);
      if (low.split2)
        for (int k = 0; k < nb; k++) HFG_HIP_CHECK(hipMemsetAsync(w.A[k].p, 0, sizeof(double) * (size_t)ns[k] * ns[k], s));
      gemm_tasklist_dev(ctx, w.gtasks.p + nb, nb, nm, nm, low);
      gemm_mirror_lower_dev(ctx, w.gtasks.p + nb, nb, nm);
    }
    eig_sym_batch(ctx, w, nb, ns.data(), Xptr, nev > 0 ? nevs.data() : nullptr);
    {
      ProfScope ps(ctx, "eig_backtransform");
      std::vector<const double *> csrc;
      std::vector<double *> cdst;
      std::vector<int> cn;
      for (int k = 0; k < nb; k++) {
        const int ib = mine[c0 + k] % nblk;
        double *slotp = dBlockBufs[mine[c0 + k] / nblk] + (size_t)ib * slot;
        csrc.push_back(nev > 0 ? w.Ws[k].p : w.d[k].p);
        cdst.push_back(slotp + nmax * nmax);
        cn.push_back(nevs[k]);
      }
      copy_slices(s, csrc, cdst, cn);
      {
        ProfScope pp3(ctx, "eig_products");
        const GemmTask *last = w.gtasks.p + (w.folded ? 3 : 2) * (size_t)nb;
        if (nev > 0)
          gemm_tasklist_dev(ctx, last, nb, nm, *std::max_element(nevs.begin(), nevs.end()), {GemmTile::T64});
        else
          gemm_tasklist_dev(ctx, last, nb, nm, nm, w.full_how);
      }
    }
    check_status(ctx, w, nb);
  }
  HFG_HIP_CHECK(hipGetLastError());
}

static void eig_assemble_sel_dev(hfg_ctx *ctx, int N, int nblk, const int64_t *blk_ptr, const int64_t *blk_idx, const double *dBlockBuf,
                                 double *dE, double *dC, int nev);
void eig_assemble_dev(hfg_ctx *ctx, int N, int nblk, const int64_t *blk_ptr, const int64_t *blk_idx,
                      const double *dBlockBuf, double *dE, double *dC) {
  eig_assemble_sel_dev(ctx, N, nblk, blk_ptr, blk_idx, dBlockBuf, dE, dC, 0);
}
int64_t eig_sel_count(int nblk, const int64_t *blk_ptr, int64_t nev) { return helfem::eig_sel_count(nblk, blk_ptr, nev); }
static void eig_assemble_sel_dev(hfg_ctx *ctx, int N, int nblk, const int64_t *blk_ptr, const int64_t *blk_idx, const double *dBlockBuf,
                                 double *dE, double *dC, int nev) {
  EigWork &w = work_for(ctx);
  hipStream_t s = ctx->stream;
  ProfScope ps(ctx, "scatter");
  if (w.asm_rows.size() != (size_t)N || !std::equal(w.asm_rows.begin(), w.asm_rows.end(), blk_idx)) {
    w.asm_rows.assign(blk_idx, blk_idx + N);
    w.asm_rows_dev.resize((size_t)N + 2);
    HFG_HIP_CHECK(hipMemcpyAsync(w.asm_rows_dev.p, w.asm_rows.data(), sizeof(int64_t) * N, hipMemcpyHostToDevice, s));
  }
  int64_t *drows = (int64_t *)w.asm_rows_dev.p;
  size_t nmax = 0;
  for (int ib = 0; ib < nblk; ib++) nmax = std::max<size_t>(nmax, blk_ptr[ib + 1] - blk_ptr[ib]);
  const size_t slot = nmax * nmax + nmax;
  DevBuf<double> &Etmp = ctx->ws[3];
  Etmp.resize(N);
  std::vector<int64_t> koff(nblk + 1, 0);
  for (int ib = 0; ib < nblk; ib++) {
    const int64_t n = blk_ptr[ib + 1] - blk_ptr[ib];
    koff[ib + 1] = koff[ib] + (nev > 0 ? std::min<int64_t>(nev, n) : n);
  }
  const int K = (int)koff[nblk];
  {
    std::vector<const double *> csrc;
    std::vector<double *> cdst;
    std::vector<int> cn;
    for (int ib = 0; ib < nblk; ib++) {
      csrc.push_back(dBlockBuf + (size_t)ib * slot + nmax * nmax);
      cdst.push_back(Etmp.p + koff[ib]);
      cn.push_back((int)(koff[ib + 1] - koff[ib]));
    }
    copy_slices(s, csrc, cdst, cn);
  }
  DevBuf<int> &rank = w.ibuf1;
  rank.resize(N + 8);
  HFG_HIP_CHECK(hipMemsetAsync(dC, 0, sizeof(double) * (size_t)N * K, s));
  launch_rank(ctx, Etmp.p, K, rank.p);
  for (int ib = 0; ib < nblk; ib++) {
    int n = (int)(blk_ptr[ib + 1] - blk_ptr[ib]), nc = (int)(koff[ib + 1] - koff[ib]);
    hipLaunchKernelGGL(k_scatter_cols, dim3((n + 255) / 256, nc), dim3(256), 0, s, dBlockBuf + (size_t)ib * slot, n, nc,
                       drows + blk_ptr[ib], rank.p, (int)koff[ib], Etmp.p + koff[ib], N, dC, dE);
  }
  HFG_HIP_CHECK(hipGetLastError());
}

void eig_gsym_sub_dev(hfg_ctx *ctx, int N, const double *dF, const double *dS, int nblk, const int64_t *blk_ptr,
                      const int64_t *blk_idx, double *dE, double *dC) {
  int save_rank = ctx->shard_rank, save_n = ctx->shard_n;
  ctx->shard_rank = 0;
  ctx->shard_n = 1;
  try {
    DevBuf<double> &buf = ctx->ws[6];
    buf.resize(eig_block_buf_size(nblk, blk_ptr));
    eig_blocks_dev(ctx, N, dF, dS, nblk, blk_ptr, blk_idx, buf.p);
    eig_assemble_dev(ctx, N, nblk, blk_ptr, blk_idx, buf.p, dE, dC);
  } catch (...) {
    ctx->shard_rank = save_rank;
    ctx->shard_n = save_n;
    throw;
  }
  ctx->shard_rank = save_rank;
  ctx->shard_n = save_n;
}

void eig_gsym_sub_sel_dev(hfg_ctx *ctx, int N, const double *dF, const double *dS, int nblk, const int64_t *blk_ptr,
                          const int64_t *blk_idx, int nev, double *dE, double *dC) {
  if (nev < 1) throw std::logic_error("eig_gsym_sub_sel: nev must be at least 1\n");
  int save_rank = ctx->shard_rank, save_n = ctx->shard_n;
  ctx->shard_rank = 0;
  ctx->shard_n = 1;
  try {
    DevBuf<double> &buf = ctx->ws[6];
    buf.resize(eig_block_buf_size(nblk, blk_ptr));
    eig_blocks_multi_dev(ctx, N, 1, &dF, dS, nblk, blk_ptr, blk_idx, &buf.p, nev);
    eig_assemble_sel_dev(ctx, N, nblk, blk_ptr, blk_idx, buf.p, dE, dC, nev);
  } catch (...) {
    ctx->shard_rank = save_rank;
    ctx->shard_n = save_n;
    throw;
  }
  ctx->shard_rank = save_rank;
  ctx->shard_n = save_n;
}

void eig_block_supports(hfg_ctx *ctx, int N, const double *dS, int nblk, const int64_t *blk_ptr, const int64_t *blk_idx,
                        std::vector<int64_t> &cols) {
  hipStream_t s = ctx->stream;
  DevBuf<int64_t> drows;
  DevBuf<int> flag;
  drows.resize(N);
  flag.resize((size_t)N * nblk + 8);
  HFG_HIP_CHECK(hipMemcpyAsync(drows.p, blk_idx, sizeof(int64_t) * N, hipMemcpyHostToDevice, s));
  for (int ib = 0; ib < nblk; ib++) {
    const int n = (int)(blk_ptr[ib + 1] - blk_ptr[ib]);
    hipLaunchKernelGGL(k_col_support, dim3(N), dim3(256), 0, s, dS, N, drows.p + blk_ptr[ib], n, flag.p + (size_t)ib * N);
  }
  std::vector<int> hflag((size_t)N * nblk);
  HFG_HIP_CHECK(hipMemcpyAsync(hflag.data(), flag.p, sizeof(int) * hflag.size(), hipMemcpyDeviceToHost, s));
  HFG_HIP_CHECK(hipStreamSynchronize(s));
  cols.clear();
  for (int ib = 0; ib < nblk; ib++) {
    int cnt = 0;
    for (int c = 0; c < N; c++)
      if (hflag[(size_t)ib * N + c]) {
        cols.push_back(c);
        cnt++;
      }
    if (cnt != (int)(blk_ptr[ib + 1] - blk_ptr[ib]))
      throw std::logic_error("eig_gsym_sub: Sinvh is not block structured (columns with support != block size)\n");
  }
}

void eig_gsym_sub_pair_dev(hfg_ctx *ctx, int N, const double *dFa, const double *dFb, const double *dS, int nblk, const int64_t *blk_ptr,
                           const int64_t *blk_idx, double *dEa, double *dCa, double *dEb, double *dCb) {
  int save_rank = ctx->shard_rank, save_n = ctx->shard_n;
  ctx->shard_rank = 0;
  ctx->shard_n = 1;
  try {
    const size_t sz = eig_block_buf_size(nblk, blk_ptr);
    DevBuf<double> &buf = ctx->ws[6];
    buf.resize(2 * sz);
    const double *Fs[2] = {dFa, dFb};
    double *bufs[2] = {buf.p, buf.p + sz};
    eig_blocks_multi_dev(ctx, N, 2, Fs, dS, nblk, blk_ptr, blk_idx, bufs);
    eig_assemble_dev(ctx, N, nblk, blk_ptr, blk_idx, bufs[0], dEa, dCa);
    eig_assemble_dev(ctx, N, nblk, blk_ptr, blk_idx, bufs[1], dEb, dCb);
  } catch (...) {
    ctx->shard_rank = save_rank;
    ctx->shard_n = save_n;
    throw;
  }
  ctx->shard_rank = save_rank;
  ctx->shard_n = save_n;
}

}
```

helfem_amd/csrc/hip/gemm.hip:

```cpp
#include "internal.h"
#include <algorithm>
#include <cstdint>
#include <cstdlib>
#include <cstring>

namespace hfg {

typedef double double4_t __attribute__((ext_vector_type(4)));
typedef double d2_t __attribute__((ext_vector_type(2)));

template <int BM, int BN, bool ACC = false, int MF = 1, bool MAP = false>
__device__ __forceinline__ void dgemm_tile(int id, int transA, int transB, int M, int N, int K, double alpha,
                                           const double *__restrict__ A, int lda, const double *__restrict__ B, int ldb,
                                           double beta, double *__restrict__ C, int ldc, double (*As)[16][BM + 16],
                                           double (*Bs)[16][BN + 16], int sym = 0, int kbeg = 0, int kend = -1, int over = 0,
                                           const int *__restrict__ amap = nullptr, const int *__restrict__ cmap = nullptr) {
  constexpr int BK = 16;
  constexpr int PAD = 16;
  constexpr int WM = BM / 2, WN = BN / 2;
  constexpr int TM = WM / 16, TN = WN / 16;
  static_assert(PAD == 16, "LDS row padding is part of the tile types");

  int nbm = (M + BM - 1) / BM, nbn = (N + BN - 1) / BN;
  const bool lower = !ACC && sym == 1;
  int nwg = lower ? nbm * (nbm + 1) / 2 : nbm * nbn;
  if (!(over & 4)) {
    int q = nwg / 8, r = nwg % 8, xcd = id % 8;
    id = (xcd < r ? xcd * (q + 1) : r * (q + 1) + (xcd - r) * q) + id / 8;
  }
  int bm = (id % nbm) * BM, bn = (id / nbm) * BN;
  if (lower) {
    int ti = (int)((sqrt(8.0 * (double)id + 1.0) - 1.0) * 0.5);
    while (ti * (ti + 1) / 2 > id) ti--;
    while ((ti + 1) * (ti + 2) / 2 <= id) ti++;
    const int tj = id - ti * (ti + 1) / 2;
    if (ti >= nbm) return;
    bm = ti * BM;
    bn = tj * BN;
  }

  if constexpr (ACC) {
    if (sym == 2 && bm / BM + 3 < bn / BN) return;
  }
  const int tid = threadIdx.x, wave = tid >> 6, lane = tid & 63;
  const int wm = (wave & 1) * WM, wn = (wave >> 1) * WN;
  const int l15 = lane & 15, l4 = lane >> 4;

  constexpr bool V4 = (MF == 1);
  double4_t accv[V4 ? TM : 1][V4 ? TN : 1];
  double accs[V4 ? 1 : TM][V4 ? 1 : TN][4];
  if constexpr (V4) {
#pragma unroll
    for (int i = 0; i < TM; i++)
#pragma unroll
      for (int j = 0; j < TN; j++) accv[i][j] = (double4_t){0.0, 0.0, 0.0, 0.0};
  } else {
#pragma unroll
    for (int i = 0; i < TM; i++)
#pragma unroll
      for (int j = 0; j < TN; j++)
#pragma unroll
        for (int c = 0; c < 4; c++) accs[i][j][c] = 0.0;
  }
  auto acc = [&](int i, int j, int r) -> double {
    if constexpr (V4) return accv[i][j][r];
    else return accs[i][j][r];
  };

  constexpr bool PRE = ACC && (TM * TN <= 4);
  double cpre[PRE ? TM : 1][PRE ? TN : 1][4];
  if constexpr (PRE) {
#pragma unroll
    for (int i = 0; i < TM; i++)
#pragma unroll
      for (int j = 0; j < TN; j++)
#pragma unroll
        for (int r = 0; r < 4; r++) {
          int gm = min(bm + wm + i * 16 + l15, M - 1), gn = min(bn + wn + j * 16 + l4 + 4 * r, N - 1);
          cpre[i][j][r] = C[(size_t)gn * ldc + gm];
        }
  }

  constexpr int VA = BM * BK / 2 / 256, VB = BN * BK / 2 / 256;
  const bool fastA = ((reinterpret_cast<uintptr_t>(A) & 15) == 0) && ((lda & 1) == 0) && (bm + BM <= M || (over & 1));
  const bool fastB = ((reinterpret_cast<uintptr_t>(B) & 15) == 0) && ((ldb & 1) == 0) && (bn + BN <= N || (over & 2));
  const int a_mv = tid % (BM / 2), a_kc = tid / (BM / 2);
  const int a_m = tid % BM, a_kv = tid / BM;
  const int b_nv = tid % (BN / 2), b_kc = tid / (BN / 2);
  const int b_n = tid % BN, b_kv = tid / BN;
  const double *pA = MAP ? A + bm + 2 * a_mv : transA ? A + (size_t)(bm + a_m) * lda + 2 * a_kv : A + (size_t)a_kc * lda + bm + 2 * a_mv;
  const double *pB = transB ? B + (size_t)b_kc * ldb + bn + 2 * b_nv : B + (size_t)(bn + b_n) * ldb + 2 * b_kv;
  d2_t va[VA], vb[VB];
  auto load_tiles = [&](int k0) {
    const bool fullk = (k0 + BK <= K);
    if constexpr (MAP) {
      if (fastA && fullk) {
#pragma unroll
        for (int r = 0; r < VA; r++) va[r] = *reinterpret_cast<const d2_t *>(pA + (size_t)amap[k0 + a_kc + r * (512 / BM)] * lda);
      } else {
#pragma unroll
        for (int r = 0; r < VA; r++) {
          const int gm0 = bm + 2 * a_mv, gk = k0 + a_kc + r * (512 / BM);
          d2_t v = (d2_t){0.0, 0.0};
          if (gk < K) {
            const double *col = A + (size_t)amap[gk] * lda;
            if (gm0 < M) v.x = col[gm0];
            if (gm0 + 1 < M) v.y = col[gm0 + 1];
          }
          va[r] = v;
        }
      }
    } else if (fastA && fullk) {
      if (!transA) {
#pragma unroll
        for (int r = 0; r < VA; r++) va[r] = *reinterpret_cast<const d2_t *>(pA + (size_t)(k0 + r * (512 / BM)) * lda);
      } else {
#pragma unroll
        for (int r = 0; r < VA; r++) va[r] = *reinterpret_cast<const d2_t *>(pA + k0 + 2 * r * (256 / BM));
      }
    } else {
#pragma unroll
      for (int r = 0; r < VA; r++) {
        int gm0, gk0, gm1, gk1;
        if (!transA) {
          gm0 = bm + 2 * a_mv;
          gm1 = gm0 + 1;
          gk0 = gk1 = k0 + a_kc + r * (512 / BM);
        } else {
          gm0 = gm1 = bm + a_m;
          gk0 = k0 + 2 * (a_kv + r * (256 / BM));
          gk1 = gk0 + 1;
        }
        d2_t v;
        v.x = (gm0 < M && gk0 < K) ? (transA ? A[(size_t)gm0 * lda + gk0] : A[(size_t)gk0 * lda + gm0]) : 0.0;
        v.y = (gm1 < M && gk1 < K) ? (transA ? A[(size_t)gm1 * lda + gk1] : A[(size_t)gk1 * lda + gm1]) : 0.0;
        va[r] = v;
      }
    }
    if (fastB && fullk) {
      if (transB) {
#pragma unroll
        for (int r = 0; r < VB; r++) vb[r] = *reinterpret_cast<const d2_t *>(pB + (size_t)(k0 + r * (512 / BN)) * ldb);
      } else {
#pragma unroll
        for (int r = 0; r < VB; r++) vb[r] = *reinterpret_cast<const d2_t *>(pB + k0 + 2 * r * (256 / BN));
      }
    } else {
#pragma unroll
      for (int r = 0; r < VB; r++) {
        int gn0, gk0, gn1, gk1;
        if (transB) {
          gn0 = bn + 2 * b_nv;
          gn1 = gn0 + 1;
          gk0 = gk1 = k0 + b_kc + r * (512 / BN);
        } else {
          gn0 = gn1 = bn + b_n;
          gk0 = k0 + 2 * (b_kv + r * (256 / BN));
          gk1 = gk0 + 1;
        }
        d2_t v;
        v.x = (gn0 < N && gk0 < K) ? (transB ? B[(size_t)gk0 * ldb + gn0] : B[(size_t)gn0 * ldb + gk0]) : 0.0;
        v.y = (gn1 < N && gk1 < K) ? (transB ? B[(size_t)gk1 * ldb + gn1] : B[(size_t)gn1 * ldb + gk1]) : 0.0;
        vb[r] = v;
      }
    }
  };
  auto store_tiles = [&](int buf) {
    if (!transA) {
#pragma unroll
      for (int r = 0; r < VA; r++) *reinterpret_cast<d2_t *>(&As[buf][a_kc + r * (512 / BM)][2 * a_mv]) = va[r];
    } else {
#pragma unroll
      for (int r = 0; r < VA; r++) {
        As[buf][2 * (a_kv + r * (256 / BM))][a_m] = va[r].x;
        As[buf][2 * (a_kv + r * (256 / BM)) + 1][a_m] = va[r].y;
      }
    }
    if (transB) {
#pragma unroll
      for (int r = 0; r < VB; r++) *reinterpret_cast<d2_t *>(&Bs[buf][b_kc + r * (512 / BN)][2 * b_nv]) = vb[r];
    } else {
#pragma unroll
      for (int r = 0; r < VB; r++) {
        Bs[buf][2 * (b_kv + r * (256 / BN))][b_n] = vb[r].x;
        Bs[buf][2 * (b_kv + r * (256 / BN)) + 1][b_n] = vb[r].y;
      }
    }
  };

  const bool splitk = kend >= 0;
  const int kstop = splitk ? min(kend, K) : K;
  load_tiles(kbeg);
  store_tiles(0);
  __syncthreads();
  int buf = 0;
  for (int k0 = kbeg; k0 < kstop; k0 += BK) {
    const bool more = (k0 + BK < kstop);
    if (more) load_tiles(k0 + BK);
#pragma unroll
    for (int kk = 0; kk < BK; kk += 4) {
      double fa[TM];
#pragma unroll
      for (int i = 0; i < TM; i++) fa[i] = As[buf][kk + l4][wm + i * 16 + l15];
      if constexpr (MF == 1) {
        double fb[TN];
#pragma unroll
        for (int j = 0; j < TN; j++) fb[j] = Bs[buf][kk + l4][wn + j * 16 + l15];
#pragma unroll
        for (int i = 0; i < TM; i++)
#pragma unroll
          for (int j = 0; j < TN; j++)
            accv[i][j] = __builtin_amdgcn_mfma_f64_16x16x4f64(fb[j], fa[i], accv[i][j], 0, 0, 0);
      } else {
#pragma unroll
        for (int j = 0; j < TN; j++) {
          double fb[4];
#pragma unroll
          for (int c = 0; c < 4; c++) fb[c] = Bs[buf][kk + l4][wn + j * 16 + 4 * c + (lane & 3)];
#pragma unroll
          for (int i = 0; i < TM; i++)
#pragma unroll
            for (int c = 0; c < 4; c++)
              accs[i][j][c] = __builtin_amdgcn_mfma_f64_4x4x4f64(fb[c], fa[i], accs[i][j][c], 0, 0, 0);
        }
      }
    }
    if (more) store_tiles(buf ^ 1);
    __syncthreads();
    buf ^= 1;
  }
  if constexpr (PRE) {
#pragma unroll
    for (int i = 0; i < TM; i++)
#pragma unroll
      for (int j = 0; j < TN; j++)
#pragma unroll
        for (int r = 0; r < 4; r++) {
          int gm = bm + wm + i * 16 + l15, gn = bn + wn + j * 16 + l4 + 4 * r;
          if (gm < M && gn < N) C[(size_t)gn * ldc + gm] = alpha * acc(i, j, r) + beta * cpre[i][j][r];
        }
    return;
  } else if constexpr (ACC) {
    constexpr int HI = (TM > 2) ? TM / 2 : TM;
#pragma unroll
    for (int i0 = 0; i0 < TM; i0 += HI) {
      double cv[HI][TN][4];
#pragma unroll
      for (int i = 0; i < HI; i++)
#pragma unroll
        for (int j = 0; j < TN; j++)
#pragma unroll
          for (int r = 0; r < 4; r++) {
            int gm = min(bm + wm + (i0 + i) * 16 + l15, M - 1), gn = min(bn + wn + j * 16 + l4 + 4 * r, N - 1);
            cv[i][j][r] = C[(size_t)gn * ldc + gm];
          }
#pragma unroll
      for (int i = 0; i < HI; i++)
#pragma unroll
        for (int j = 0; j < TN; j++)
#pragma unroll
          for (int r = 0; r < 4; r++) {
            int gm = bm + wm + (i0 + i) * 16 + l15, gn = bn + wn + j * 16 + l4 + 4 * r;
            if (gm < M && gn < N) C[(size_t)gn * ldc + gm] = alpha * acc(i0 + i, j, r) + beta * cv[i][j][r];
          }
    }
    return;
  }
#pragma unroll
  for (int i = 0; i < TM; i++)
#pragma unroll
    for (int j = 0; j < TN; j++)
#pragma unroll
      for (int r = 0; r < 4; r++) {
        int gm = bm + wm + i * 16 + l15, gn = bn + wn + j * 16 + l4 + 4 * r;
        if (gm < M && gn < N) {
          size_t o;
          if constexpr (MAP) o = (size_t)cmap[gn] * ldc + gm;
          else o = (size_t)gn * ldc + gm;
          double v = alpha * acc(i, j, r);
          if (splitk) {
            unsafeAtomicAdd(&C[o], v);
            continue;
          }
          if (beta != 0.0) v += beta * C[o];
          C[o] = v;
        }
      }
}

template <int BM, int BN, int MF = 1>
__global__ __launch_bounds__(256, 2) void k_dgemm(int transA, int transB, int M, int N, int K, double alpha,
                                               const double *__restrict__ A, int lda, const double *__restrict__ B,
                                               int ldb, double beta, double *__restrict__ C, int ldc) {
  __shared__ __attribute__((aligned(16))) double As[2][16][BM + 16];
  __shared__ __attribute__((aligned(16))) double Bs[2][16][BN + 16];
  dgemm_tile<BM, BN, false, MF>(blockIdx.x, transA, transB, M, N, K, alpha, A, lda, B, ldb, beta, C, ldc, As, Bs);
}

template <int BM, int BN, bool ACC = false, int MF = 1>
__global__ __launch_bounds__(256, 2) void k_dgemm_tasklist(const GemmTask *__restrict__ tasks) {
  __shared__ __attribute__((aligned(16))) double As[2][16][BM + 16];
  __shared__ __attribute__((aligned(16))) double Bs[2][16][BN + 16];
  const GemmTask t = tasks[blockIdx.y];
  if (t.M <= 0 || t.N <= 0) return;
  const int sym = (!ACC && BM == BN && t.M == t.N && t.beta == 0.0) ? (t.sym == 1) : ((ACC && t.sym == 2) ? 2 : 0);
  const int nbm = (t.M + BM - 1) / BM;
  const int nt = (sym == 1) ? nbm * (nbm + 1) / 2 : nbm * ((t.N + BN - 1) / BN);
  if ((int)blockIdx.x >= nt) return;
  dgemm_tile<BM, BN, ACC, MF>(blockIdx.x, t.tA, t.tB, t.M, t.N, t.K, t.alpha, t.A, t.lda, t.B, t.ldb, t.beta, t.C, t.ldc,
                              As, Bs, sym, 0, -1, t.over);
}

template <int MF = 1>
__global__ __launch_bounds__(256, 2) void k_dgemm_tasklist_map(const GemmTask *__restrict__ tasks) {
  __shared__ __attribute__((aligned(16))) double As[2][16][64 + 16];
  __shared__ __attribute__((aligned(16))) double Bs[2][16][64 + 16];
  const GemmTask t = tasks[blockIdx.y];
  if (t.M <= 0 || t.N <= 0) return;
  const int nt = ((t.M + 63) / 64) * ((t.N + 63) / 64);
  if ((int)blockIdx.x >= nt) return;
  dgemm_tile<64, 64, false, MF, true>(blockIdx.x, 0, 0, t.M, t.N, t.K, t.alpha, t.A, t.lda, t.B, t.ldb, 0.0, t.C, t.ldc, As, Bs, 0,
                                      0, -1, 0, t.amap, t.cmap);
}

template <int BM, int BN, bool SPLIT = false>
__global__ __launch_bounds__(256, 2) void k_dgemm_tasklist_wl(const GemmTask *__restrict__ tasks, const int2 *__restrict__ wl, int nwg) {
  __shared__ __attribute__((aligned(16))) double As[2][16][BM + 16];
  __shared__ __attribute__((aligned(16))) double Bs[2][16][BN + 16];
  const int xcd = blockIdx.x % 8, slot = blockIdx.x / 8;
  const int q8 = nwg / 8, r8 = nwg % 8;
  if (slot >= q8 + (xcd < r8 ? 1 : 0)) return;
  const int2 w = wl[(xcd < r8 ? xcd * (q8 + 1) : r8 * (q8 + 1) + (xcd - r8) * q8) + slot];
  const GemmTask t = tasks[w.x];
  if constexpr (SPLIT) {
    const int half = w.y & 1;
    const int Kh = ((t.K / 2 + 15) / 16) * 16;
    const int kbeg = half ? Kh : 0, kend = half ? t.K : Kh;
    if (kbeg >= kend) return;
    dgemm_tile<BM, BN, false, 1>(w.y >> 1, t.tA, t.tB, t.M, t.N, t.K, t.alpha, t.A, t.lda, t.B, t.ldb, 0.0, t.C, t.ldc, As, Bs, 0, kbeg,
                                 kend, t.over | 4);
  } else {
    dgemm_tile<BM, BN, false, 1>(w.y, t.tA, t.tB, t.M, t.N, t.K, t.alpha, t.A, t.lda, t.B, t.ldb, t.beta, t.C, t.ldc, As, Bs, 0, 0, -1,
                                 t.over | 4);
  }
}

template <int BM, int BN>
__global__ __launch_bounds__(256, 2) void k_dgemm_tasklist_split2(const GemmTask *__restrict__ tasks) {
  __shared__ __attribute__((aligned(16))) double As[2][16][BM + 16];
  __shared__ __attribute__((aligned(16))) double Bs[2][16][BN + 16];
  const GemmTask t = tasks[blockIdx.y];
  if (t.M <= 0 || t.N <= 0) return;
  const int sym = (BM == BN && t.M == t.N) ? (t.sym == 1) : 0;
  const int nbm = (t.M + BM - 1) / BM;
  const int nt = (sym == 1) ? nbm * (nbm + 1) / 2 : nbm * ((t.N + BN - 1) / BN);
  const int tile = blockIdx.x >> 1, half = blockIdx.x & 1;
  if (tile >= nt) return;
  const int Kh = ((t.K / 2 + 15) / 16) * 16;
  const int kbeg = half ? Kh : 0, kend = half ? t.K : Kh;
  if (kbeg >= kend) return;
  dgemm_tile<BM, BN, false, 1>(tile, t.tA, t.tB, t.M, t.N, t.K, t.alpha, t.A, t.lda, t.B, t.ldb, 0.0, t.C, t.ldc, As, Bs, sym, kbeg, kend);
}

__global__ __launch_bounds__(256) void k_mirror_lower(const GemmTask *__restrict__ tasks) {
  __shared__ double tile[64][65];
  const GemmTask t = tasks[blockIdx.y];
  if (t.sym != 1 || t.M <= 0 || t.M != t.N) return;
  const int nb = (t.M + 63) / 64;
  int bi = (int)((1.0 + sqrt(1.0 + 8.0 * (double)blockIdx.x)) * 0.5);
  while (bi * (bi - 1) / 2 > (int)blockIdx.x) bi--;
  while ((bi + 1) * bi / 2 <= (int)blockIdx.x) bi++;
  const int bj = blockIdx.x - bi * (bi - 1) / 2;
  if (bi >= nb) return;
  const int tx = threadIdx.x & 63, ty = threadIdx.x >> 6;
  for (int c = ty; c < 64; c += 4) {
    int gm = bi * 64 + tx, gn = bj * 64 + c;
    tile[c][tx] = (gm < t.M && gn < t.N) ? t.C[(size_t)gn * t.ldc + gm] : 0.0;
  }
  __syncthreads();
  for (int c = ty; c < 64; c += 4) {
    int gm = bj * 64 + tx, gn = bi * 64 + c;
    if (gm < t.M && gn < t.N) t.C[(size_t)gn * t.ldc + gm] = tile[tx][c];
  }
}

void gemm_mirror_lower_dev(hfg_ctx *ctx, const GemmTask *dtasks, int ntasks, int maxN) {
  if (ntasks <= 0 || maxN <= 64) return;
  const int nb = (maxN + 63) / 64;
  hipLaunchKernelGGL(k_mirror_lower, dim3(nb * (nb - 1) / 2, ntasks), dim3(256), 0, ctx->stream, dtasks);
  HFG_HIP_CHECK(hipGetLastError());
}

static bool mfma4() { return tuning().mfma_4x4x4; }

namespace {
struct TileShape {
  int bm, bn;
};
TileShape tile_shape(GemmTile tile) {
  switch (tile) {
    case GemmTile::T64: return {64, 64};
    case GemmTile::T128: return {128, 128};
    case GemmTile::T128x64: return {128, 64};
    default: throw std::logic_error("GEMM tile engine: GemmTile::Auto names no tile shape");
  }
}
int tile_count(TileShape s, int M, int N) { return ((M + s.bm - 1) / s.bm) * ((N + s.bn - 1) / s.bn); }
const char *tile_name(GemmTile tile) {
  const char *names[] = {"Auto", "T64", "T128", "T128x64"};
  return (unsigned)tile < 4u ? names[(int)tile] : "(unknown)";
}

typedef void (*TaskKernel)(const GemmTask *);
constexpr int ACC = 1, SPLIT2 = 2, MAP = 4;
constexpr int variant(GemmTile tile, int flags) { return 8 * (int)tile + flags; }
TaskKernel tasklist_kernel(GemmTile tile, const GemmHow &how) {
  const bool m4 = mfma4();
  switch (variant(tile, how.acc * ACC + how.split2 * SPLIT2 + how.map * MAP)) {
    case variant(GemmTile::T64, 0): return m4 ? k_dgemm_tasklist<64, 64, false, 0> : k_dgemm_tasklist<64, 64>;
    case variant(GemmTile::T128, 0): return m4 ? k_dgemm_tasklist<128, 128, false, 0> : k_dgemm_tasklist<128, 128>;
    case variant(GemmTile::T128x64, 0): return k_dgemm_tasklist<128, 64>;
    case variant(GemmTile::T64, ACC): return m4 ? k_dgemm_tasklist<64, 64, true, 0> : k_dgemm_tasklist<64, 64, true>;
    case variant(GemmTile::T128, ACC): return m4 ? k_dgemm_tasklist<128, 128, true, 0> : k_dgemm_tasklist<128, 128, true>;
    case variant(GemmTile::T64, MAP): return m4 ? k_dgemm_tasklist_map<0> : k_dgemm_tasklist_map<1>;
    case variant(GemmTile::T128, SPLIT2): return k_dgemm_tasklist_split2<128, 128>;
    case variant(GemmTile::T128x64, SPLIT2): return k_dgemm_tasklist_split2<128, 64>;
    default:
      throw std::logic_error(std::string("gemm_tasklist_dev: no kernel for tile ") + tile_name(tile) + (how.acc ? " acc" : "") +
                             (how.split2 ? " split2" : "") + (how.map ? " map" : ""));
  }
}
}

void gemm_tasklist_dev(hfg_ctx *ctx, const GemmTask *dtasks, int ntasks, int maxM, int maxN, GemmHow how) {
  if (ntasks <= 0 || maxM <= 0 || maxN <= 0) return;
  GemmTile tile = how.tile;
  if (tile == GemmTile::Auto)
    tile = (ntasks <= 65535 && !gemm_prefers_128(ctx, (long)ntasks * tile_count({128, 128}, maxM, maxN))) ? GemmTile::T64 : GemmTile::T128;
  const TaskKernel kernel = tasklist_kernel(tile, how);
  const int tiles = tile_count(tile_shape(tile), maxM, maxN) * (how.split2 ? 2 : 1);
  ProfScope ps(ctx, "gemm");
  for (int t0 = 0; t0 < ntasks; t0 += 65535)
    hipLaunchKernelGGL(kernel, dim3(tiles, std::min(65535, ntasks - t0)), dim3(256), 0, ctx->stream, dtasks + t0);
  HFG_HIP_CHECK(hipGetLastError());
}

void gemm_worklist(const std::vector<GemmTask> &tasks, GemmTile tile, bool split2, std::vector<int2> &out) {
  const TileShape shape = tile_shape(tile);
  out.clear();
  for (size_t t = 0; t < tasks.size(); t++) {
    if (tasks[t].M <= 0 || tasks[t].N <= 0) continue;
    const int n = tile_count(shape, tasks[t].M, tasks[t].N) * (split2 ? 2 : 1);
    for (int q = 0; q < n; q++) out.push_back(make_int2((int)t, q));
  }
}

void gemm_worklist_dev(hfg_ctx *ctx, const GemmTask *dtasks, const int2 *dwl, int nwg, GemmTile tile, bool split2) {
  void (*kernel)(const GemmTask *, const int2 *, int) = nullptr;
  if (split2) {
    if (tile == GemmTile::T128x64) kernel = k_dgemm_tasklist_wl<128, 64, true>;
  } else if (tile == GemmTile::T128) kernel = k_dgemm_tasklist_wl<128, 128>;
  else if (tile == GemmTile::T128x64) kernel = k_dgemm_tasklist_wl<128, 64>;
  else if (tile == GemmTile::T64) kernel = k_dgemm_tasklist_wl<64, 64>;
  if (!kernel) throw std::logic_error(std::string("gemm_worklist_dev: no kernel for tile ") + tile_name(tile) + (split2 ? " split2" : ""));
  if (nwg <= 0) return;
  ProfScope ps(ctx, "gemm");
  hipLaunchKernelGGL(kernel, dim3(8u * (unsigned)((nwg + 7) / 8)), dim3(256), 0, ctx->stream, dtasks, dwl, nwg);
  HFG_HIP_CHECK(hipGetLastError());
}

bool gemm_prefers_128(hfg_ctx *ctx, long tiles128) {
  if (tuning().gemm_tile) return tuning().gemm_tile == 128;
  static const int slots = [&] {
    int ncu = 256;
    (void)hipDeviceGetAttribute(&ncu, hipDeviceAttributeMultiprocessorCount, ctx->device);
    return 2 * ncu;
  }();
  const long rounds = (tiles128 + slots - 1) / slots;
  return tiles128 >= slots / 2 && (double)tiles128 >= 0.85 * (double)(rounds * slots);
}

void gemm_dev(hfg_ctx *ctx, bool tA, bool tB, int M, int N, int K, double alpha, const double *A, int lda,
              const double *B, int ldb, double beta, double *C, int ldc) {
  if (M <= 0 || N <= 0) return;
  ProfScope ps(ctx, "gemm");
  const long big_tiles = (long)((M + 127) / 128) * ((N + 127) / 128);
  const bool big = gemm_prefers_128(ctx, big_tiles), m4 = mfma4();
  const long tiles = big ? big_tiles : (long)((M + 63) / 64) * ((N + 63) / 64);
  const auto kernel = big ? (m4 ? k_dgemm<128, 128, 0> : k_dgemm<128, 128>) : (m4 ? k_dgemm<64, 64, 0> : k_dgemm<64, 64>);
  hipLaunchKernelGGL(kernel, dim3((unsigned)tiles), dim3(256), 0, ctx->stream, (int)tA, (int)tB, M, N, K, alpha, A, lda, B, ldb, beta, C,
                     ldc);
  HFG_HIP_CHECK(hipGetLastError());
}

}
```

helfem_amd/csrc/hip/internal.h:

```cpp
#pragma once
#include "common.h"
#include "tables.h"
#include "../host/scf.h"

namespace hfg {

enum class GemmTile { Auto, T64, T128, T128x64 };
struct GemmHow {
  GemmTile tile = GemmTile::Auto;
  bool acc = false, split2 = false, map = false;
};
void gemm_tasklist_dev(hfg_ctx *ctx, const GemmTask *dtasks, int ntasks, int maxM, int maxN, GemmHow how = {});
void gemm_worklist_dev(hfg_ctx *ctx, const GemmTask *dtasks, const int2 *dwl, int nwg, GemmTile tile, bool split2 = false);
void gemm_worklist(const std::vector<GemmTask> &tasks, GemmTile tile, bool split2, std::vector<int2> &out);
void gemm_mirror_lower_dev(hfg_ctx *ctx, const GemmTask *dtasks, int ntasks, int maxN);
bool gemm_prefers_128(hfg_ctx *ctx, long tiles128);
void gemm_dev(hfg_ctx *ctx, bool tA, bool tB, int M, int N, int K, double alpha, const double *A, int lda, const double *B, int ldb,
              double beta, double *C, int ldc);

void coulomb_dev(hfg_ctx *ctx, hfg_basis *basis, const double *dP, double *dJ);
void coulomb_batch_dev(hfg_ctx *ctx, hfg_basis *basis, int64_t nP, const double *dP, double *dJ);
void coulomb_energy_matrix_dev(hfg_ctx *ctx, hfg_basis *basis, int64_t nP, const double *dP, double *dW);
void set_xc_params(hfg_ctx *ctx, int x_func, const double *x_pars, int nx, int c_func, const double *c_pars, int nc);
void xc_eval_host(int id, int nspin, size_t np, const double *rho, const double *sigma, const double *lapl, const double *tau,
                  double *exc, double *vrho, double *vsigma, double *vlapl, double *vtau, double thr);
void xc_eval_host_ext(int id, const double *pars, int npars, int nspin, size_t np, const double *rho, const double *sigma,
                      const double *lapl, const double *tau, double *exc, double *vrho, double *vsigma, double *vlapl, double *vtau,
                      double thr);
void xc_fock_dev(hfg_ctx *ctx, hfg_basis *basis, int x_func, int c_func, const double *dP, double *dH, double *dScal,
                 double thr);
void xc_fock_pol_dev(hfg_ctx *ctx, hfg_basis *basis, int x_func, int c_func, const double *dPa, const double *dPb, double *dHa,
                     double *dHb, double *dScal, double thr);
void model_potential_dev(hfg_ctx *ctx, hfg_basis *basis, int kind1, int Z1, double d1, double H1, int kind2, int Z2, double d2,
                         double H2, double *dH);
void set_fock_blocks(hfg_ctx *ctx, hfg_basis *basis, const int *dBlockId);
size_t fock_compact_size(hfg_basis *basis);
void fock_compact_dev(hfg_ctx *ctx, hfg_basis *basis, int x_func, int c_func, const double *dP, double *dFc, double *dScal,
                      double thr);
void fock_finish_dev(hfg_ctx *ctx, hfg_basis *basis, const double *dFc, const double *dH0, const int *dBlockId,
                     double *dF);
void fock_compact_pol_dev(hfg_ctx *ctx, hfg_basis *basis, int x_func, int c_func, const double *dPa, const double *dPb,
                          double *dFc, double *dScal, double thr);
void fock_finish_pol_dev(hfg_ctx *ctx, hfg_basis *basis, const double *dFc, const double *dH0, const int *dBlockId,
                         double *dFa, double *dFb);

void exchange_dev(hfg_ctx *ctx, hfg_basis *basis, const double *dP, double *dK, bool rs = false, const double *Lknown = nullptr,
                  int rknown = 0);
bool exchange_lowrank_dev(hfg_ctx *ctx, hfg_dev_tables *t, const double *dP, double *dK, const double *Lknown,
                          int rknown);
void exchange_batch_dev(hfg_ctx *ctx, hfg_basis *basis, int64_t nP, const double *dP, double *dK, bool rs = false,
                        const double *dC = nullptr, const int64_t *nocc = nullptr, int64_t ldc = 0);

void compute_tei_dev(hfg_ctx *ctx, hfg_basis *basis);

void compute_rs_tei_dev(hfg_ctx *ctx, hfg_basis *basis, int rs_kind, double omega);
void rs_special_dev(hfg_ctx *ctx, int which, int L, const double *a, const double *b, size_t n, double *out);

void eig_sym_dev(hfg_ctx *ctx, int n, const double *dA, double *dE, double *dC);
void eig_gsym_dev(hfg_ctx *ctx, int N, int n, const double *dF, const double *dS, double *dE, double *dC);
void eig_gsym_sub_dev(hfg_ctx *ctx, int N, const double *dF, const double *dS, int nblk, const int64_t *blk_ptr,
                      const int64_t *blk_idx, double *dE, double *dC);
void eig_gsym_sub_pair_dev(hfg_ctx *ctx, int N, const double *dFa, const double *dFb, const double *dS, int nblk,
                           const int64_t *blk_ptr, const int64_t *blk_idx, double *dEa, double *dCa, double *dEb,
                           double *dCb);
size_t eig_block_buf_size(int nblk, const int64_t *blk_ptr);
void eig_blocks_dev(hfg_ctx *ctx, int N, const double *dF, const double *dS, int nblk, const int64_t *blk_ptr,
                    const int64_t *blk_idx, double *dBlockBuf);
void eig_assemble_dev(hfg_ctx *ctx, int N, int nblk, const int64_t *blk_ptr, const int64_t *blk_idx, const double *dBlockBuf,
                      double *dE, double *dC);
void eig_block_supports(hfg_ctx *ctx, int N, const double *dS, int nblk, const int64_t *blk_ptr, const int64_t *blk_idx,
                        std::vector<int64_t> &cols);
int64_t eig_sel_count(int nblk, const int64_t *blk_ptr, int64_t nev);
void eig_sym_sel_dev(hfg_ctx *ctx, int n, const double *dA, int nev, double *dE, double *dC);
void eig_gsym_sub_sel_dev(hfg_ctx *ctx, int N, const double *dF, const double *dS, int nblk, const int64_t *blk_ptr,
                          const int64_t *blk_idx, int nev, double *dE, double *dC);

void tridiag_dc_batch(hfg_ctx *ctx, int nblk, const int *ns, double *const *d, double *const *e, double *const *Z);
int dc_status(hfg_ctx *ctx);
int *dc_status_word(hfg_ctx *ctx);
void tridiag_sel_batch(hfg_ctx *ctx, int nblk, const int *ns, const int *nev, double *const *d, double *const *e, double *const *W,
                       double *const *Z);
void tridiagonalize_batch(hfg_ctx *ctx, int nblk, const int *ns, double *const *A, double *const *d, double *const *e,
                          double *const *tau);
void trd_measure_gemv(hfg_ctx *ctx, double *ms, int64_t *launches);
bool tridiagonalize_takes_chain(int nblk, const int *ns);
void tridiagonalize_persistent(hfg_ctx *ctx, int nblk, const int *ns, double *const *A, double *const *d, double *const *e,
                               double *const *tau, std::vector<char> &done);
void trdp_check_status(hfg_ctx *ctx);

void form_sinvh_dev(hfg_ctx *ctx, int N, const double *dS, bool chol, int nblk, const int64_t *blk_ptr, const int64_t *blk_idx,
                    double *dSinvh);
void form_density_dev(hfg_ctx *ctx, int N, int ncols, const double *dC, int nocc, double *dP);

constexpr int DIIS_LR_MAXCOLS = 64;
constexpr int DIIS_HIST_CHUNK = 8;
struct DiisErrTask {
  const double *A, *B;
  double *out;
  int n, k, ld, ldo;
};
struct DiisHistory {
  const double *E[DIIS_HIST_CHUNK], *P[DIIS_HIST_CHUNK], *F[DIIS_HIST_CHUNK];
  int n;
};
struct DiisComb {
  const double *F[16];
  double w[16];
  int n;
};
size_t diis_lowrank_partials(int ntasks, int nmax);
void diis_lowrank_error_dev(hfg_ctx *ctx, const DiisErrTask *dtasks, int ntasks, int nmax, double *dPartialMax,
                            double *dMax);
void diis_history_dev(hfg_ctx *ctx, const DiisHistory &h, int j0, int nhtot, const double *dEnew, size_t elen, const double *dPnew,
                      const double *dFnew, size_t flen, bool want_max, double *dPartial, double *dRes);
void diis_extrapolate_dev(hfg_ctx *ctx, const DiisComb &c, size_t NN, int nspin, double *dFa, double *dFb);

helfem::scf::Result scf_device_loop(hfg_ctx *ctx, hfg_basis *hb, const helfem::scf::Options &opt, int nel, double Enucr, int symm,
                                    const std::vector<std::vector<size_t> > &dsym, int ldft, int mdft,
                                    const std::vector<std::vector<std::vector<size_t> > > &avg_idx =
                                        std::vector<std::vector<std::vector<size_t> > >());

}
```

helfem_amd/csrc/host/tuning.h:

```cpp
#pragma once
#include <string>

namespace helfem {
constexpr int EXL_GMAX = 16;
enum class TrdMode { persistent, chain, twokernel, unblocked };
enum class EigSel { crossover, stein, dc };
enum class RsTei { host, dev };
#define HELFEM_TUNING(X) \
  X(scf_host, bool, false, "HELFEM_SCF", true, "=host", !strcmp(e, "host"), "SCF loop driven from the host through the per-stage entry points (checker of the device-resident loop)") \
  X(tei_host, bool, false, "HELFEM_TEI", false, "=host", !strcmp(e, "host"), "in-element tables built by the threaded host code and uploaded (checker of tei_dev.hip)") \
  X(rs_tei, RsTei, RsTei::host, "HELFEM_RS_TEI", false, "word", !strcmp(e, "dev") ? RsTei::dev : RsTei::host, "range-separated exchange tables of the SCF drivers: dev = built on the device (rs_tei_dev.hip); unset or any other word = built by the threaded host code and uploaded") \
  X(exchange_general, bool, false, "HELFEM_EXCHANGE", true, "=general", !strcmp(e, "general"), "general exchange kernels always, not only where the low-rank fast path declines") \
  X(exl_rb, int, 0, "HELFEM_EXL_RB", false, "int", atoi(e), "RB kernel of the low-rank exchange: 4 the 4 x 4 vector kernel, 1 the one-pair vector kernel (checkers), else the matrix-core kernel k_exl_RBm") \
  X(exl_mgroups, bool, true, "HELFEM_EXL_MGROUPS", false, "off if 0", atoi(e) != 0, "cross-element products by blocks of equal m; off: the full products") \
  X(exl_rect, int, -1, "HELFEM_EXL_RECT", false, "int", atoi(e), "tiles of the element GEMM: 0 / 1 / 2 = 128 x 128 / 128 x 64 / 64 x 64 always; negative: 64 x 64 when the tasks average fewer than 1500 pairs, else 128 x 128") \
  X(exl_wl, bool, true, "HELFEM_EXL_WL", false, "off if 0", atoi(e) != 0, "XCD-contiguous workgroup lists for the element GEMM and the cross products; off: plain task-list grids") \
  X(exl_splitk, bool, true, "HELFEM_EXL_SPLITK", false, "off if 0", atoi(e) != 0, "two half-K workgroups per tile for the cross products; off: one workgroup per tile") \
  X(exl_crect, bool, true, "HELFEM_EXL_CRECT", false, "off if 0", atoi(e) != 0, "128 x 64 tiles for the split cross products; off: 128 x 128") \
  X(exl_groups, int, 4, "HELFEM_EXL_GROUPS", false, "int", std::max(1, std::min(EXL_GMAX, atoi(e))), "groups of 64 factors tried before the general kernels take over, clamped to 1 ... 16") \
  X(exl_hint, bool, true, "HELFEM_EXL_HINT", false, "off if 0", atoi(e) != 0, "the SCF loop's occupied orbitals taken as the factors of P; off: always factorise and verify P (checker)") \
  X(exl_pair, bool, true, "HELFEM_EXL_PAIR", false, "off if 0", atoi(e) != 0, "low-rank fast path for the pair (erfc) tables; off: general kernels") \
  X(fock_overlap, bool, true, "HELFEM_FOCK_OVERLAP", false, "off if 0", atoi(e) != 0, "Coulomb kernels on the side stream beside the XC kernels; off: one after the other on the main stream") \
  X(fock_skip, bool, true, "HELFEM_FOCK_SKIP", true, "off if 0", atoi(e) != 0, "Fock build skips shell pairs whose density block is zero and, after hfg_ctx_set_fock_blocks, pairs the caller does not read; off: every pair is computed (checker)") \
  X(xc_lds_limit, size_t, 150 * 1024, "HELFEM_XC_LDS_LIMIT", false, "int", (size_t)atol(e), "bytes of LDS the angular XC kernels plan with; smaller forces the chunked kernels (tests)") \
  X(coulomb_batch_chunk, int, 0, "HELFEM_COULOMB_BATCH_CHUNK", true, "int", std::max(0, atoi(e)), "densities per pass over the tables of the batched Coulomb build forced smaller than the LDS rule allows (tests; 0: the rule's own)") \
  X(exchange_batch_chunk, int, 0, "HELFEM_EXCHANGE_BATCH_CHUNK", true, "int", std::max(0, atoi(e)), "densities per pass over the tables of the batched exchange build at most (tests; 0: as many as fit the 64 factor columns of a pass)") \
  X(uscf_kbatch, bool, false, "HELFEM_USCF_KBATCH", true, "=1", atoi(e) == 1, "DeviceUSCFStep: K[Pa] and K[Pb] through one call of hfg_exchange_occ_batch_devptr; off: one call per spin") \
  X(diis_blocks, bool, true, "HELFEM_DIIS_BLOCKS", false, "off if 0", atoi(e) != 0, "DIIS error per symmetry block; off: the four dense N^3 products (checker)") \
  X(diis_lowrank, bool, true, "HELFEM_DIIS_LOWRANK", false, "off if 0", atoi(e) != 0, "blocked DIIS error from the occupied orbitals; off: per-block n^3 products from F and P (checker)") \
  X(eig_pair, bool, true, "HELFEM_EIG_PAIR", false, "off if 0", atoi(e) != 0, "both spins' Fock matrices in one batched eigensolve; off: two calls") \
  X(trd_mode, TrdMode, TrdMode::persistent, "HELFEM_TRD", false, "word", !strcmp(e, "persistent") ? TrdMode::persistent : !strcmp(e, "twokernel") ? TrdMode::twokernel : !strcmp(e, "unblocked") ? TrdMode::unblocked : TrdMode::chain, "tridiagonalisation: persistent = k_trdp where the batch fits, else the chain; chain (and any unknown word) = one k_trdf launch per column always (checker); twokernel = k_trdb_gemv + k_trdb_w; unblocked = the first-generation kernels") \
  X(trdp_min, int, 256, "HELFEM_TRDP_MIN", false, "int", atoi(e), "smallest order the persistent kernel takes") \
  X(trdp_r, int, 0, "HELFEM_TRDP_R", false, "int", atoi(e), "rows per thread of the persistent kernel forced (0: the first that fits)") \
  X(trdp_u, int, 0, "HELFEM_TRDP_U", false, "int", atoi(e), "column chunks per thread of the persistent kernel forced wider than needed (measurement; 0: narrowest)") \
  X(trdp_limit_ms, long long, 200, "HELFEM_TRDP_LIMIT_MS", false, "int", atoll(e), "wall-clock bound of every spin of the persistent kernel, ms") \
  X(trdp_phases, bool, true, "HELFEM_TRDP_PHASES", false, "off if 0", atoi(e) != 0, "one cooperative launch per phase; off: the whole matrix in one launch (checker)") \
  X(trdp_step, int, 96, "HELFEM_TRDP_STEP", false, "int", std::max(1, atoi(e)), "fewest columns of a phase (at least 1)") \
  X(trdp_coop, bool, true, "HELFEM_TRDP_COOP", false, "off if 0", atoi(e) != 0, "hipLaunchCooperativeKernel for the phases; off: plain launches (A/B of the launch overhead)") \
  X(trdp_stamps, int, 0, "HELFEM_TRDP_STAMPS", false, "int", atoi(e), "non-zero: the stamping kernels, one launch per eigensolve, phase summary on stderr; 2 and more: also per-column stamps of one workgroup") \
  X(trdp_stamps_file, std::string, "", "HELFEM_TRDP_STAMPS_FILE", false, "path", e, "with stamps: file for the stamps of every workgroup over 64 columns (tools/trdp_window.py)") \
  X(trd_tail, int, 2, "HELFEM_TRD_TAIL", false, "int", atoi(e), "last columns of the chain in one launch: 0 none, 1 the LDS-resident kernel (order 128), else the register-resident kernel (order 192)") \
  X(trdf_sym, int, -1, "HELFEM_TRDF_SYM", false, "int", atoi(e), "symmetric sweep of k_trdf: 0 never, other non-negative always, negative by HELFEM_TRDF_SYM_MIN") \
  X(trdf_sym_min, int, 0, "HELFEM_TRDF_SYM_MIN", false, "int", atoi(e), "panels whose full grid has more tiles than this sweep one triangle only") \
  X(trd_band_update, bool, true, "HELFEM_TRD_BAND_UPDATE", false, "off if 0", atoi(e) != 0, "band-limited trailing updates when every sweep is symmetric; off: full updates") \
  X(trdf_nth, int, 0, "HELFEM_TRDF_NTH", false, "int", atoi(e), "512: k_trdf with 512 threads; anything else 1024 (A/B runs)") \
  X(acc_tile, int, 0, "HELFEM_ACC_TILE", false, "int", atoi(e), "128: 128 x 128 tiles for the accumulating updates (and full, not band-limited ones); anything else 64 x 64") \
  X(trdf_dbg, int, 0, "HELFEM_TRDF_DBG", false, "int", atoi(e), "measurement replay of k_trdf only: bits 0-2 go to the kernel's debug field, bit 2 also prints the per-wave stamps (tools/trdf_probe.py)") \
  X(trdf_c, int, -1, "HELFEM_TRDF_C", false, "int", atoi(e), "measurement replay of k_trdf only: column-in-panel index forced for every launch (negative: each launch's own)") \
  X(tridiag_ql, bool, false, "HELFEM_TRIDIAG", false, "=ql", !strcmp(e, "ql"), "one-lane implicit QL for the tridiagonal problem instead of divide and conquer (checker)") \
  X(dc_gemm_small, bool, false, "HELFEM_DC_GEMM", false, "=small", !strcmp(e, "small"), "Q U of the divide-and-conquer merges by the first 64 x 64 kernel instead of the tile engine (checker)") \
  X(dc_levels, bool, false, "HELFEM_DC", false, "=levels", !strcmp(e, "levels"), "divide-and-conquer merges with the gather, scatter and copy-back passes over Q and ten launches per level (checker of the column-mapped product)") \
  X(eigsel, EigSel, EigSel::crossover, "HELFEM_EIGSEL", false, "word", !strcmp(e, "stein") ? EigSel::stein : !strcmp(e, "dc") ? EigSel::dc : EigSel::crossover, "selected eigenpairs (hfg_eig_*_sel): stein = multisection and inverse iteration always; dc = the full divide and conquer, then the lowest columns (checker); unset or any other word = the crossover, which sends every wanted fraction to dc (measured: stein is slower down to 1/64 of the columns)") \
  X(dc_dbg, bool, false, "HELFEM_DC_DBG", false, "present", true, "merge statistics of divide and conquer on stderr") \
  X(bt_column, bool, false, "HELFEM_BT", false, "=column", !strcmp(e, "column"), "back-transformation reflector by reflector instead of compact WY (checker)") \
  X(bt_fold, bool, true, "HELFEM_BT_FOLD", false, "off if 0", atoi(e) != 0, "X Q formed on the side stream beside divide and conquer; off: Z <- Q Z on the main stream behind it") \
  X(bt_side, bool, false, "HELFEM_BT_SIDE", false, "=1", atoi(e) == 1, "without the fold: the compact-WY set-up on the side stream") \
  X(gemm_tile, int, 0, "HELFEM_GEMM_TILE", false, "int", atoi(e), "128: 128 x 128 tiles always; other non-zero: 64 x 64 always; 0: the large tiles where they fill whole rounds of the chip") \
  X(gemm_splitk, int, -1, "HELFEM_GEMM_SPLITK", false, "int", atoi(e), "eigensolve's products: 0 / other non-negative = large tiles without / with two half-K workgroups each; negative: chosen by tile count") \
  X(gemm_rect, bool, false, "HELFEM_GEMM_RECT", false, "on if not 0", atoi(e) != 0, "128 x 64 tiles for the eigensolve's large-tile products") \
  X(mfma_4x4x4, bool, false, "HELFEM_MFMA", false, "=4x4x4", !strcmp(e, "4x4x4"), "v_mfma_f64_4x4x4_4b_f64 in the tile engine instead of v_mfma_f64_16x16x4_f64 (A/B runs)") \
  X(num_threads, int, 0, "HELFEM_NUM_THREADS", true, "int", std::max(0, atoi(e)), "host threads of the set-up code (0: one per core, 64 at most)") \
  X(hdf5_lib, std::string, "", "HELFEM_HDF5_LIB", true, "path", e, "HDF5 library tried before the usual names")

struct Tuning {
#define X(field, type, def, ...) type field = def;
  HELFEM_TUNING(X)
#undef X
};
const Tuning &tuning();
Tuning tuning_live();
std::string tuning_table();
}
```

Measured before the change: 8.068 ms.

## Store blocked eigenvectors straight into C and cache the S-derived X blocks

On a single rank the SCF step now calls one blocked eigensolve that ranks eigenvalues before the final back-transform. A scatter GEMM variant then writes each block's product directly into the sorted columns of the full C matrix through row and column maps, which skips the block-slot buffer, the memset and the separate assemble pass. The per-block X gathered from the overlap is kept across calls when S is unchanged, so later iterations gather only F. It adds new kernel variants, a pinned status readback, and a full memset of C before the scatter.

```diff
diff --git a/helfem_amd/__init__.py b/helfem_amd/__init__.py
--- a/helfem_amd/__init__.py
+++ b/helfem_amd/__init__.py
@@ -1196,6 +1196,11 @@
                                           self.blk_ptr.ctypes.data_as(c_i64_p), self.blk_idx.ctypes.data_as(c_i64_p),
                                           self._ptr(self.blockbuf), self._ptr(self.E), self._ptr(self.C)))
 
+    def eig_whole(self):
+        _check(lib().hfg_eig_gsym_sub_dev(self.ctx.h, ctypes.c_int64(self.N), self._ptr(self.F), self._ptr(self.Sinvh),
+                                          len(self.blocks), self.blk_ptr.ctypes.data_as(c_i64_p),
+                                          self.blk_idx.ctypes.data_as(c_i64_p), self._ptr(self.E), self._ptr(self.C)))
+
     def density(self):
         _check(lib().hfg_form_density_dev(self.ctx.h, ctypes.c_int64(self.N), ctypes.c_int64(self.N), self._ptr(self.C),
                                           ctypes.c_int64(self.nocc), self._ptr(self.P)))
@@ -1217,12 +1222,7 @@
             if allreduce is not None:
                 allreduce(self.K)
             self.F.add_(self.K, alpha=self.kfrac)
-        self.eig_partial()
-        if exchange_blocks is not None:
-            exchange_blocks(self.blockbuf, len(self.blocks))
-        elif allreduce is not None:
-            allreduce(self.blockbuf)
-        self.eig_finish()
+        self._eig_stage(allreduce, exchange_blocks)
         self.density()
         self.have_C = True
 
@@ -1255,6 +1255,9 @@
         self.F.add_(self.K, alpha=self.kfrac)
 
     def _eig_stage(self, allreduce, exchange_blocks):
+        if self.nranks == 1 and allreduce is None and exchange_blocks is None:
+            self.eig_whole()
+            return
         self.eig_partial()
         if exchange_blocks is not None:
             exchange_blocks(self.blockbuf, len(self.blocks))
diff --git a/helfem_amd/csrc/hip/common.h b/helfem_amd/csrc/hip/common.h
--- a/helfem_amd/csrc/hip/common.h
+++ b/helfem_amd/csrc/hip/common.h
@@ -138,8 +138,9 @@
   int sym = 0;
   int over = 0;
   const int *amap = nullptr, *cmap = nullptr;
+  const int64_t *rmap = nullptr;
 };
-static_assert(sizeof(GemmTask) == 96, "GemmTask is compared bytewise: keep it free of padding");
+static_assert(sizeof(GemmTask) == 104, "GemmTask is compared bytewise: keep it free of padding");
 
 struct ProfScope {
   hfg_ctx *c;
diff --git a/helfem_amd/csrc/hip/eig.hip b/helfem_amd/csrc/hip/eig.hip
--- a/helfem_amd/csrc/hip/eig.hip
+++ b/helfem_amd/csrc/hip/eig.hip
@@ -3,6 +3,7 @@
 #include "../host/eigsel_count.h"
 #include <cstdlib>
 #include <cstring>
+#include <functional>
 
 namespace hfg {
 
@@ -34,6 +35,13 @@
   if (i >= n) return;
   Fb[(size_t)j * n + i] = F[(size_t)rows[j] * N + rows[i]];
   Xb[(size_t)j * n + i] = S[(size_t)cols[j] * N + rows[i]];
+}
+
+__global__ void k_gather_f(const double *__restrict__ F, int N, const int64_t *__restrict__ rows, int n, double *__restrict__ Fb) {
+  int i = blockIdx.x * blockDim.x + threadIdx.x;
+  int j = blockIdx.y;
+  if (i >= n) return;
+  Fb[(size_t)j * n + i] = F[(size_t)rows[j] * N + rows[i]];
 }
 
 __global__ void k_col_support(const double *__restrict__ S, int N, const int64_t *__restrict__ rows, int n,
@@ -389,6 +397,11 @@
   hipLaunchKernelGGL(k_rank, dim3((n + 255) / 256, RANK_SEG), dim3(256), 0, ctx->stream, E, n, rank);
 }
 
+__global__ void k_place_values(const double *__restrict__ E, int n, const int *__restrict__ rank, double *__restrict__ Eout) {
+  int i = blockIdx.x * blockDim.x + threadIdx.x;
+  if (i < n) Eout[rank[i]] = E[i];
+}
+
 __global__ void k_scatter_cols(const double *__restrict__ Cb, int nrow, int ncol, const int64_t *__restrict__ rows,
                                const int *__restrict__ rank, int coff, const double *__restrict__ Eb, int ldc,
                                double *__restrict__ Cout, double *__restrict__ Eout) {
@@ -587,6 +600,14 @@
   unsigned long sup_gen = 0;
   int sup_N = 0;
   std::vector<int64_t> sup_ptr, sup_idx;
+  DevBuf<double> Xc;
+  std::vector<char> xc_have;
+  int *h_status = nullptr;
+  hipEvent_t status_ev = nullptr;
+  ~EigWork() {
+    if (h_status) (void)hipHostFree(h_status);
+    if (status_ev) (void)hipEventDestroy(status_ev);
+  }
 };
 static EigWork &work_for(hfg_ctx *ctx) { return ctx->work.get<EigWork>(WS_EIG); }
 
@@ -890,7 +911,7 @@
   return (double)want <= EIGSEL_CROSS * (double)all;
 }
 static void eig_sym_batch(hfg_ctx *ctx, EigWork &w, int nblk, const int *ns, const double *const *foldX = nullptr,
-                          const int *nev = nullptr) {
+                          const int *nev = nullptr, const std::function<void()> &after_solve = nullptr) {
   EigBatch b;
   b.nblk = nblk;
   int nmax = 0, nzmax = 0;
@@ -1008,6 +1029,7 @@
       }
     }
   }
+  if (after_solve) after_solve();
   {
     ProfScope ps(ctx, "eig_backtransform");
     if (fold) {
@@ -1104,7 +1126,8 @@
 }
 
 static void eig_blocks_multi_dev(hfg_ctx *ctx, int N, int nF, const double *const *dFs, const double *dS, int nblk, const int64_t *blk_ptr,
-                                 const int64_t *blk_idx, double *const *dBlockBufs, int nev = 0);
+                                 const int64_t *blk_idx, double *const *dBlockBufs, int nev = 0, double *const *dEs = nullptr,
+                                 double *const *dCs = nullptr);
 static int eig_num_cus(hfg_ctx *ctx) {
   static const int ncu = [&] {
     hipDeviceProp_t prop;
@@ -1117,9 +1140,11 @@
   eig_blocks_multi_dev(ctx, N, 1, &dF, dS, nblk, blk_ptr, blk_idx, &dBlockBuf);
 }
 static void eig_blocks_multi_dev(hfg_ctx *ctx, int N, int nF, const double *const *dFs, const double *dS, int nblk, const int64_t *blk_ptr,
-                                 const int64_t *blk_idx, double *const *dBlockBufs, int nev) {
+                                 const int64_t *blk_idx, double *const *dBlockBufs, int nev, double *const *dEs, double *const *dCs) {
   EigWork &w = work_for(ctx);
   hipStream_t s = ctx->stream;
+  const bool direct = dEs != nullptr;
+  if (direct && (ctx->shard_n != 1 || nF * nblk > MAXB)) throw std::logic_error("eig_blocks_multi_dev: direct path needs one rank and one batch\n");
   if (blk_ptr[nblk] != N) throw std::logic_error("Symmetry mismatch in eig_gsym_sub\n");
   DevBuf<double> &idxbuf = w.idx;
   idxbuf.resize(2 * (size_t)N + 16);
@@ -1133,6 +1158,7 @@
                       w.sup_idx.size() == (size_t)N && std::equal(w.sup_idx.begin(), w.sup_idx.end(), blk_idx);
   if (!cached) {
     w.sup_S = nullptr;
+    w.xc_have.clear();
     HFG_HIP_CHECK(hipMemcpyAsync(drows, blk_idx, sizeof(int64_t) * N, hipMemcpyHostToDevice, s));
     DevBuf<int> &flag = w.ibuf2;
     flag.resize((size_t)N * nblk + 8);
@@ -1168,7 +1194,29 @@
   size_t nmax = 0;
   for (int ib = 0; ib < nblk; ib++) nmax = std::max<size_t>(nmax, blk_ptr[ib + 1] - blk_ptr[ib]);
   const size_t slot = nmax * nmax + nmax;
-  for (int f = 0; f < nF; f++) HFG_HIP_CHECK(hipMemsetAsync(dBlockBufs[f], 0, sizeof(double) * slot * nblk, s));
+  if (!direct && ctx->shard_n > 1)
+    for (int f = 0; f < nF; f++) HFG_HIP_CHECK(hipMemsetAsync(dBlockBufs[f], 0, sizeof(double) * slot * nblk, s));
+  const bool keep_x = w.sup_S == dS && w.sup_S != nullptr;
+  std::vector<size_t> xoff(nblk + 1, 0);
+  for (int ib = 0; ib < nblk; ib++) xoff[ib + 1] = xoff[ib] + (size_t)(blk_ptr[ib + 1] - blk_ptr[ib]) * (size_t)(blk_ptr[ib + 1] - blk_ptr[ib]);
+  if (keep_x) {
+    if (w.xc_have.size() != (size_t)nblk || w.Xc.n < xoff[nblk]) {
+      w.Xc.resize(xoff[nblk]);
+      w.xc_have.assign(nblk, 0);
+    }
+  }
+  std::vector<int64_t> koff(nblk + 1, 0);
+  for (int ib = 0; ib < nblk; ib++) {
+    const int64_t n = blk_ptr[ib + 1] - blk_ptr[ib];
+    koff[ib + 1] = koff[ib] + (nev > 0 ? std::min<int64_t>(nev, n) : n);
+  }
+  const int K = (int)koff[nblk];
+  DevBuf<int> &rank = w.ibuf1;
+  DevBuf<double> &Etmp = ctx->ws[3];
+  if (direct) {
+    rank.resize((size_t)nF * (N + 8));
+    Etmp.resize((size_t)nF * N);
+  }
 
   std::vector<int> mine;
   for (int f = 0; f < nF; f++)
@@ -1188,7 +1236,7 @@
     int nm = 0;
     for (int k = 0; k < nb; k++) {
       const int ib = mine[c0 + k] % nblk;
-      double *dBlockBuf = dBlockBufs[mine[c0 + k] / nblk];
+      double *dBlockBuf = direct ? nullptr : dBlockBufs[mine[c0 + k] / nblk];
       int n = (int)(blk_ptr[ib + 1] - blk_ptr[ib]);
       ns[k] = n;
       nevs[k] = nev > 0 ? std::min(nev, n) : n;
@@ -1197,7 +1245,8 @@
       if (nev > 0) w.Zs[k].resize((size_t)n * nevs[k]);
       else w.Z[k].resize((size_t)n * n);
       w.Y[k].resize((size_t)n * n);
-      double *Xb = Xall.p + (size_t)k * nmax * nmax, *Fk = Fb.p + (size_t)k * nmax * nmax, *Tk = T1.p + (size_t)k * nmax * nmax;
+      double *Xb = keep_x ? w.Xc.p + xoff[ib] : Xall.p + (size_t)k * nmax * nmax;
+      double *Fk = Fb.p + (size_t)k * nmax * nmax, *Tk = T1.p + (size_t)k * nmax * nmax;
       Xptr[k] = Xb;
       GemmTask g;
       g.M = g.N = g.K = n;
@@ -1217,7 +1266,14 @@
       g.A = Xb;
       g.B = nev > 0 ? w.Zs[k].p : w.Z[k].p;
       g.N = nevs[k];
-      g.C = dBlockBuf + (size_t)ib * slot;
+      if (direct) {
+        const int f = mine[c0 + k] / nblk;
+        g.C = dCs[f];
+        g.ldc = N;
+        g.rmap = drows + blk_ptr[ib];
+        g.cmap = rank.p + (size_t)f * (N + 8) + koff[ib];
+      } else
+        g.C = dBlockBuf + (size_t)ib * slot;
       gt[2 * nb + k] = g;
       g.A = w.Y[k].p;
       g.tA = 1;
@@ -1230,8 +1286,12 @@
         const int ib = mine[c0 + k] % nblk;
         const double *dF = dFs[mine[c0 + k] / nblk];
         int n = ns[k];
-        hipLaunchKernelGGL(k_gather_block, dim3((n + 255) / 256, n), dim3(256), 0, s, dF, dS, N, drows + blk_ptr[ib],
-                           dcols + blk_ptr[ib], n, Fb.p + (size_t)k * nmax * nmax, Xall.p + (size_t)k * nmax * nmax);
+        if (keep_x && w.xc_have[ib])
+          hipLaunchKernelGGL(k_gather_f, dim3((n + 255) / 256, n), dim3(256), 0, s, dF, N, drows + blk_ptr[ib], n, Fb.p + (size_t)k * nmax * nmax);
+        else
+          hipLaunchKernelGGL(k_gather_block, dim3((n + 255) / 256, n), dim3(256), 0, s, dF, dS, N, drows + blk_ptr[ib],
+                             dcols + blk_ptr[ib], n, Fb.p + (size_t)k * nmax * nmax, const_cast<double *>(Xptr[k]));
+        if (keep_x) w.xc_have[ib] = 1;
       }
       const int force_split = tuning().gemm_splitk;
       long full_tiles = 0, low_tiles = 0;
@@ -1261,29 +1321,64 @@
       gemm_tasklist_dev(ctx, w.gtasks.p + nb, nb, nm, nm, low);
       gemm_mirror_lower_dev(ctx, w.gtasks.p + nb, nb, nm);
     }
-    eig_sym_batch(ctx, w, nb, ns.data(), Xptr, nev > 0 ? nevs.data() : nullptr);
+    std::function<void()> after_solve;
+    if (direct)
+      after_solve = [&] {
+        if (w.used_dc) {
+          if (!w.h_status) HFG_HIP_CHECK(hipHostMalloc((void **)&w.h_status, sizeof(int), hipHostMallocDefault));
+          if (!w.status_ev) HFG_HIP_CHECK(hipEventCreateWithFlags(&w.status_ev, hipEventDisableTiming));
+          HFG_HIP_CHECK(hipMemcpyAsync(w.h_status, dc_status_word(ctx), sizeof(int), hipMemcpyDeviceToHost, s));
+          HFG_HIP_CHECK(hipEventRecord(w.status_ev, s));
+        }
+        ProfScope ps(ctx, "scatter");
+        std::vector<const double *> csrc;
+        std::vector<double *> cdst;
+        std::vector<int> cn;
+        for (int k = 0; k < nb; k++) {
+          const int ib = mine[c0 + k] % nblk, f = mine[c0 + k] / nblk;
+          csrc.push_back(nev > 0 ? w.Ws[k].p : w.d[k].p);
+          cdst.push_back(Etmp.p + (size_t)f * N + koff[ib]);
+          cn.push_back(nevs[k]);
+        }
+        copy_slices(s, csrc, cdst, cn);
+        for (int f = 0; f < nF; f++) {
+          int *rk = rank.p + (size_t)f * (N + 8);
+          launch_rank(ctx, Etmp.p + (size_t)f * N, K, rk);
+          hipLaunchKernelGGL(k_place_values, dim3((K + 255) / 256), dim3(256), 0, s, Etmp.p + (size_t)f * N, K, rk, dEs[f]);
+          HFG_HIP_CHECK(hipMemsetAsync(dCs[f], 0, sizeof(double) * (size_t)N * K, s));
+        }
+      };
+    eig_sym_batch(ctx, w, nb, ns.data(), Xptr, nev > 0 ? nevs.data() : nullptr, after_solve);
     {
       ProfScope ps(ctx, "eig_backtransform");
-      std::vector<const double *> csrc;
-      std::vector<double *> cdst;
-      std::vector<int> cn;
-      for (int k = 0; k < nb; k++) {
-        const int ib = mine[c0 + k] % nblk;
-        double *slotp = dBlockBufs[mine[c0 + k] / nblk] + (size_t)ib * slot;
-        csrc.push_back(nev > 0 ? w.Ws[k].p : w.d[k].p);
-        cdst.push_back(slotp + nmax * nmax);
-        cn.push_back(nevs[k]);
-      }
-      copy_slices(s, csrc, cdst, cn);
+      if (!direct) {
+        std::vector<const double *> csrc;
+        std::vector<double *> cdst;
+        std::vector<int> cn;
+        for (int k = 0; k < nb; k++) {
+          const int ib = mine[c0 + k] % nblk;
+          double *slotp = dBlockBufs[mine[c0 + k] / nblk] + (size_t)ib * slot;
+          csrc.push_back(nev > 0 ? w.Ws[k].p : w.d[k].p);
+          cdst.push_back(slotp + nmax * nmax);
+          cn.push_back(nevs[k]);
+          if (nev <= 0 && w.full_how.split2 && ctx->shard_n == 1)
+            HFG_HIP_CHECK(hipMemsetAsync(slotp, 0, sizeof(double) * (size_t)ns[k] * ns[k], s));
+        }
+        copy_slices(s, csrc, cdst, cn);
+      }
       {
         ProfScope pp3(ctx, "eig_products");
         const GemmTask *last = w.gtasks.p + (w.folded ? 3 : 2) * (size_t)nb;
-        if (nev > 0)
-          gemm_tasklist_dev(ctx, last, nb, nm, *std::max_element(nevs.begin(), nevs.end()), {GemmTile::T64});
-        else
-          gemm_tasklist_dev(ctx, last, nb, nm, nm, w.full_how);
-      }
-    }
+        GemmHow how = nev > 0 ? GemmHow{GemmTile::T64} : w.full_how;
+        how.scatter = direct;
+        gemm_tasklist_dev(ctx, last, nb, nm, nev > 0 ? *std::max_element(nevs.begin(), nevs.end()) : nm, how);
+      }
+    }
+    if (direct && w.used_dc) {
+      HFG_HIP_CHECK(hipEventSynchronize(w.status_ev));
+      if (*w.h_status != 0) throw std::logic_error("Eigendecomposition failed!\n");
+      trdp_check_status(ctx);
+    } else
     check_status(ctx, w, nb);
   }
   HFG_HIP_CHECK(hipGetLastError());
@@ -1341,16 +1436,24 @@
   HFG_HIP_CHECK(hipGetLastError());
 }
 
-void eig_gsym_sub_dev(hfg_ctx *ctx, int N, const double *dF, const double *dS, int nblk, const int64_t *blk_ptr,
-                      const int64_t *blk_idx, double *dE, double *dC) {
+static void eig_gsym_sub_multi_dev(hfg_ctx *ctx, int N, int nF, const double *const *dFs, const double *dS, int nblk, const int64_t *blk_ptr,
+                                   const int64_t *blk_idx, int nev, double *const *dEs, double *const *dCs) {
   int save_rank = ctx->shard_rank, save_n = ctx->shard_n;
   ctx->shard_rank = 0;
   ctx->shard_n = 1;
   try {
-    DevBuf<double> &buf = ctx->ws[6];
-    buf.resize(eig_block_buf_size(nblk, blk_ptr));
-    eig_blocks_dev(ctx, N, dF, dS, nblk, blk_ptr, blk_idx, buf.p);
-    eig_assemble_dev(ctx, N, nblk, blk_ptr, blk_idx, buf.p, dE, dC);
+    if (helfem::tuning_live().eig_direct && nF * nblk <= MAXB) {
+      eig_blocks_multi_dev(ctx, N, nF, dFs, dS, nblk, blk_ptr, blk_idx, nullptr, nev, dEs, dCs);
+    } else {
+      const size_t sz = eig_block_buf_size(nblk, blk_ptr);
+      DevBuf<double> &buf = ctx->ws[6];
+      buf.resize(nF * sz);
+      double *bufs[MAXB];
+      if (nF > MAXB) throw std::logic_error("eig_gsym_sub: too many matrices in one call\n");
+      for (int f = 0; f < nF; f++) bufs[f] = buf.p + f * sz;
+      eig_blocks_multi_dev(ctx, N, nF, dFs, dS, nblk, blk_ptr, blk_idx, bufs, nev);
+      for (int f = 0; f < nF; f++) eig_assemble_sel_dev(ctx, N, nblk, blk_ptr, blk_idx, bufs[f], dEs[f], dCs[f], nev);
+    }
   } catch (...) {
     ctx->shard_rank = save_rank;
     ctx->shard_n = save_n;
@@ -1360,24 +1463,15 @@
   ctx->shard_n = save_n;
 }
 
+void eig_gsym_sub_dev(hfg_ctx *ctx, int N, const double *dF, const double *dS, int nblk, const int64_t *blk_ptr,
+                      const int64_t *blk_idx, double *dE, double *dC) {
+  eig_gsym_sub_multi_dev(ctx, N, 1, &dF, dS, nblk, blk_ptr, blk_idx, 0, &dE, &dC);
+}
+
 void eig_gsym_sub_sel_dev(hfg_ctx *ctx, int N, const double *dF, const double *dS, int nblk, const int64_t *blk_ptr,
                           const int64_t *blk_idx, int nev, double *dE, double *dC) {
   if (nev < 1) throw std::logic_error("eig_gsym_sub_sel: nev must be at least 1\n");
-  int save_rank = ctx->shard_rank, save_n = ctx->shard_n;
-  ctx->shard_rank = 0;
-  ctx->shard_n = 1;
-  try {
-    DevBuf<double> &buf = ctx->ws[6];
-    buf.resize(eig_block_buf_size(nblk, blk_ptr));
-    eig_blocks_multi_dev(ctx, N, 1, &dF, dS, nblk, blk_ptr, blk_idx, &buf.p, nev);
-    eig_assemble_sel_dev(ctx, N, nblk, blk_ptr, blk_idx, buf.p, dE, dC, nev);
-  } catch (...) {
-    ctx->shard_rank = save_rank;
-    ctx->shard_n = save_n;
-    throw;
-  }
-  ctx->shard_rank = save_rank;
-  ctx->shard_n = save_n;
+  eig_gsym_sub_multi_dev(ctx, N, 1, &dF, dS, nblk, blk_ptr, blk_idx, nev, &dE, &dC);
 }
 
 void eig_block_supports(hfg_ctx *ctx, int N, const double *dS, int nblk, const int64_t *blk_ptr, const int64_t *blk_idx,
@@ -1410,25 +1504,9 @@
 
 void eig_gsym_sub_pair_dev(hfg_ctx *ctx, int N, const double *dFa, const double *dFb, const double *dS, int nblk, const int64_t *blk_ptr,
                            const int64_t *blk_idx, double *dEa, double *dCa, double *dEb, double *dCb) {
-  int save_rank = ctx->shard_rank, save_n = ctx->shard_n;
-  ctx->shard_rank = 0;
-  ctx->shard_n = 1;
-  try {
-    const size_t sz = eig_block_buf_size(nblk, blk_ptr);
-    DevBuf<double> &buf = ctx->ws[6];
-    buf.resize(2 * sz);
-    const double *Fs[2] = {dFa, dFb};
-    double *bufs[2] = {buf.p, buf.p + sz};
-    eig_blocks_multi_dev(ctx, N, 2, Fs, dS, nblk, blk_ptr, blk_idx, bufs);
-    eig_assemble_dev(ctx, N, nblk, blk_ptr, blk_idx, bufs[0], dEa, dCa);
-    eig_assemble_dev(ctx, N, nblk, blk_ptr, blk_idx, bufs[1], dEb, dCb);
-  } catch (...) {
-    ctx->shard_rank = save_rank;
-    ctx->shard_n = save_n;
-    throw;
-  }
-  ctx->shard_rank = save_rank;
-  ctx->shard_n = save_n;
-}
-
-}
+  const double *Fs[2] = {dFa, dFb};
+  double *Es[2] = {dEa, dEb}, *Cs[2] = {dCa, dCb};
+  eig_gsym_sub_multi_dev(ctx, N, 2, Fs, dS, nblk, blk_ptr, blk_idx, 0, Es, Cs);
+}
+
+}
diff --git a/helfem_amd/csrc/hip/gemm.hip b/helfem_amd/csrc/hip/gemm.hip
--- a/helfem_amd/csrc/hip/gemm.hip
+++ b/helfem_amd/csrc/hip/gemm.hip
@@ -9,12 +9,13 @@
 typedef double double4_t __attribute__((ext_vector_type(4)));
 typedef double d2_t __attribute__((ext_vector_type(2)));
 
-template <int BM, int BN, bool ACC = false, int MF = 1, bool MAP = false>
+template <int BM, int BN, bool ACC = false, int MF = 1, bool MAP = false, bool RMAP = false>
 __device__ __forceinline__ void dgemm_tile(int id, int transA, int transB, int M, int N, int K, double alpha,
                                            const double *__restrict__ A, int lda, const double *__restrict__ B, int ldb,
                                            double beta, double *__restrict__ C, int ldc, double (*As)[16][BM + 16],
                                            double (*Bs)[16][BN + 16], int sym = 0, int kbeg = 0, int kend = -1, int over = 0,
-                                           const int *__restrict__ amap = nullptr, const int *__restrict__ cmap = nullptr) {
+                                           const int *__restrict__ amap = nullptr, const int *__restrict__ cmap = nullptr,
+                                           const int64_t *__restrict__ rmap = nullptr) {
   constexpr int BK = 16;
   constexpr int PAD = 16;
   constexpr int WM = BM / 2, WN = BN / 2;
@@ -275,7 +276,8 @@
         int gm = bm + wm + i * 16 + l15, gn = bn + wn + j * 16 + l4 + 4 * r;
         if (gm < M && gn < N) {
           size_t o;
-          if constexpr (MAP) o = (size_t)cmap[gn] * ldc + gm;
+          if constexpr (RMAP) o = (size_t)cmap[gn] * ldc + (size_t)rmap[gm];
+          else if constexpr (MAP) o = (size_t)cmap[gn] * ldc + gm;
           else o = (size_t)gn * ldc + gm;
           double v = alpha * acc(i, j, r);
           if (splitk) {
@@ -321,6 +323,18 @@
   if ((int)blockIdx.x >= nt) return;
   dgemm_tile<64, 64, false, MF, true>(blockIdx.x, 0, 0, t.M, t.N, t.K, t.alpha, t.A, t.lda, t.B, t.ldb, 0.0, t.C, t.ldc, As, Bs, 0,
                                       0, -1, 0, t.amap, t.cmap);
+}
+
+template <int BM, int BN, int MF = 1>
+__global__ __launch_bounds__(256, 2) void k_dgemm_tasklist_scatter(const GemmTask *__restrict__ tasks) {
+  __shared__ __attribute__((aligned(16))) double As[2][16][BM + 16];
+  __shared__ __attribute__((aligned(16))) double Bs[2][16][BN + 16];
+  const GemmTask t = tasks[blockIdx.y];
+  if (t.M <= 0 || t.N <= 0) return;
+  const int nt = ((t.M + BM - 1) / BM) * ((t.N + BN - 1) / BN);
+  if ((int)blockIdx.x >= nt) return;
+  dgemm_tile<BM, BN, false, MF, false, true>(blockIdx.x, t.tA, t.tB, t.M, t.N, t.K, t.alpha, t.A, t.lda, t.B, t.ldb, 0.0, t.C, t.ldc,
+                                             As, Bs, 0, 0, -1, t.over, nullptr, t.cmap, t.rmap);
 }
 
 template <int BM, int BN, bool SPLIT = false>
@@ -361,6 +375,21 @@
   if (kbeg >= kend) return;
   dgemm_tile<BM, BN, false, 1>(tile, t.tA, t.tB, t.M, t.N, t.K, t.alpha, t.A, t.lda, t.B, t.ldb, 0.0, t.C, t.ldc, As, Bs, sym, kbeg, kend);
 }
+template <int BM, int BN>
+__global__ __launch_bounds__(256, 2) void k_dgemm_tasklist_split2_scatter(const GemmTask *__restrict__ tasks) {
+  __shared__ __attribute__((aligned(16))) double As[2][16][BM + 16];
+  __shared__ __attribute__((aligned(16))) double Bs[2][16][BN + 16];
+  const GemmTask t = tasks[blockIdx.y];
+  if (t.M <= 0 || t.N <= 0) return;
+  const int nt = ((t.M + BM - 1) / BM) * ((t.N + BN - 1) / BN);
+  const int tile = blockIdx.x >> 1, half = blockIdx.x & 1;
+  if (tile >= nt) return;
+  const int Kh = ((t.K / 2 + 15) / 16) * 16;
+  const int kbeg = half ? Kh : 0, kend = half ? t.K : Kh;
+  if (kbeg >= kend) return;
+  dgemm_tile<BM, BN, false, 1, false, true>(tile, t.tA, t.tB, t.M, t.N, t.K, t.alpha, t.A, t.lda, t.B, t.ldb, 0.0, t.C, t.ldc, As, Bs, 0,
+                                            kbeg, kend, 0, nullptr, t.cmap, t.rmap);
+}
 
 __global__ __launch_bounds__(256) void k_mirror_lower(const GemmTask *__restrict__ tasks) {
   __shared__ double tile[64][65];
@@ -412,11 +441,11 @@
 }
 
 typedef void (*TaskKernel)(const GemmTask *);
-constexpr int ACC = 1, SPLIT2 = 2, MAP = 4;
-constexpr int variant(GemmTile tile, int flags) { return 8 * (int)tile + flags; }
+constexpr int ACC = 1, SPLIT2 = 2, MAP = 4, SCATTER = 8;
+constexpr int variant(GemmTile tile, int flags) { return 16 * (int)tile + flags; }
 TaskKernel tasklist_kernel(GemmTile tile, const GemmHow &how) {
   const bool m4 = mfma4();
-  switch (variant(tile, how.acc * ACC + how.split2 * SPLIT2 + how.map * MAP)) {
+  switch (variant(tile, how.acc * ACC + how.split2 * SPLIT2 + how.map * MAP + how.scatter * SCATTER)) {
     case variant(GemmTile::T64, 0): return m4 ? k_dgemm_tasklist<64, 64, false, 0> : k_dgemm_tasklist<64, 64>;
     case variant(GemmTile::T128, 0): return m4 ? k_dgemm_tasklist<128, 128, false, 0> : k_dgemm_tasklist<128, 128>;
     case variant(GemmTile::T128x64, 0): return k_dgemm_tasklist<128, 64>;
@@ -425,9 +454,14 @@
     case variant(GemmTile::T64, MAP): return m4 ? k_dgemm_tasklist_map<0> : k_dgemm_tasklist_map<1>;
     case variant(GemmTile::T128, SPLIT2): return k_dgemm_tasklist_split2<128, 128>;
     case variant(GemmTile::T128x64, SPLIT2): return k_dgemm_tasklist_split2<128, 64>;
+    case variant(GemmTile::T64, SCATTER): return m4 ? k_dgemm_tasklist_scatter<64, 64, 0> : k_dgemm_tasklist_scatter<64, 64>;
+    case variant(GemmTile::T128, SCATTER): return m4 ? k_dgemm_tasklist_scatter<128, 128, 0> : k_dgemm_tasklist_scatter<128, 128>;
+    case variant(GemmTile::T128x64, SCATTER): return k_dgemm_tasklist_scatter<128, 64>;
+    case variant(GemmTile::T128, SPLIT2 + SCATTER): return k_dgemm_tasklist_split2_scatter<128, 128>;
+    case variant(GemmTile::T128x64, SPLIT2 + SCATTER): return k_dgemm_tasklist_split2_scatter<128, 64>;
     default:
       throw std::logic_error(std::string("gemm_tasklist_dev: no kernel for tile ") + tile_name(tile) + (how.acc ? " acc" : "") +
-                             (how.split2 ? " split2" : "") + (how.map ? " map" : ""));
+                             (how.split2 ? " split2" : "") + (how.map ? " map" : "") + (how.scatter ? " scatter" : ""));
   }
 }
 }
diff --git a/helfem_amd/csrc/hip/internal.h b/helfem_amd/csrc/hip/internal.h
--- a/helfem_amd/csrc/hip/internal.h
+++ b/helfem_amd/csrc/hip/internal.h
@@ -8,7 +8,7 @@
 enum class GemmTile { Auto, T64, T128, T128x64 };
 struct GemmHow {
   GemmTile tile = GemmTile::Auto;
-  bool acc = false, split2 = false, map = false;
+  bool acc = false, split2 = false, map = false, scatter = false;
 };
 void gemm_tasklist_dev(hfg_ctx *ctx, const GemmTask *dtasks, int ntasks, int maxM, int maxN, GemmHow how = {});
 void gemm_worklist_dev(hfg_ctx *ctx, const GemmTask *dtasks, const int2 *dwl, int nwg, GemmTile tile, bool split2 = false);
diff --git a/helfem_amd/csrc/host/tuning.h b/helfem_amd/csrc/host/tuning.h
--- a/helfem_amd/csrc/host/tuning.h
+++ b/helfem_amd/csrc/host/tuning.h
@@ -29,6 +29,7 @@
   X(diis_blocks, bool, true, "HELFEM_DIIS_BLOCKS", false, "off if 0", atoi(e) != 0, "DIIS error per symmetry block; off: the four dense N^3 products (checker)") \
   X(diis_lowrank, bool, true, "HELFEM_DIIS_LOWRANK", false, "off if 0", atoi(e) != 0, "blocked DIIS error from the occupied orbitals; off: per-block n^3 products from F and P (checker)") \
   X(eig_pair, bool, true, "HELFEM_EIG_PAIR", false, "off if 0", atoi(e) != 0, "both spins' Fock matrices in one batched eigensolve; off: two calls") \
+  X(eig_direct, bool, true, "HELFEM_EIG_DIRECT", true, "off if 0", atoi(e) != 0, "one-call blocked eigensolve (hfg_eig_gsym_sub_dev, _sel_dev, _pair_devptr) ranks before its last product and stores that product straight into C; off: block slots, then hfg_eig_assemble_dev (checker)") \
   X(trd_mode, TrdMode, TrdMode::persistent, "HELFEM_TRD", false, "word", !strcmp(e, "persistent") ? TrdMode::persistent : !strcmp(e, "twokernel") ? TrdMode::twokernel : !strcmp(e, "unblocked") ? TrdMode::unblocked : TrdMode::chain, "tridiagonalisation: persistent = k_trdp where the batch fits, else the chain; chain (and any unknown word) = one k_trdf launch per column always (checker); twokernel = k_trdb_gemv + k_trdb_w; unblocked = the first-generation kernels") \
   X(trdp_min, int, 256, "HELFEM_TRDP_MIN", false, "int", atoi(e), "smallest order the persistent kernel takes") \
   X(trdp_r, int, 0, "HELFEM_TRDP_R", false, "int", atoi(e), "rows per thread of the persistent kernel forced (0: the first that fits)") \
```

Result: faster. 7.919 ms, median of 6 (-1.8%).
